# USDA-ARS-GBRU/itsxpress

Measured on AMD Instinct MI355X. Metric: reads/sec trimmed (ITS2, stand-in taxon Tracheophyta for Fungi), higher is better.
Workload: dtype u8+f32

## Files before the change

itsxpress_amd/csrc/engine.hip:

```cpp
#include <algorithm>
#include <chrono>
#include <cmath>
#include <cstdio>
#include <cstring>
#include <functional>
#include <map>
#include <memory>
#include <numeric>
#include <atomic>
#include <condition_variable>
#include <mutex>
#include <thread>
#include "detmath.h"
#include "engine.h"
#include "k_api.h"
#include "cluster_multi.h"
#include "fastq_io.h"
#include "writers.h"

namespace itsx {
void launch_region_offsets(int64_t npairs, const PairRec *pairs, const int32_t *pref, const int64_t *seg_pair_start,
                           const int64_t *seg_region_start, int64_t *pair_region0, hipStream_t st);
void launch_finalize(itsx_domain *dom, int64_t n, const int64_t *domz, double domE, const int32_t *usample, int P, hipStream_t st);
void launch_positions(const itsx_domain *dom, int64_t n, const int8_t *side, unsigned long long *bl, unsigned long long *br,
// ... 190 lines not shown
    NameList r;
    r.blob.assign(blob.begin() + off[lo], blob.begin() + off[hi]);
    r.off.resize(hi - lo + 1);
    for (size_t i = lo; i <= hi; i++) r.off[i - lo] = off[i] - off[lo];
    return r;
  }
};

template <class T> struct DBuf {
  T *p = nullptr; size_t n = 0, cap = 0;
  int pool_device = -1;
  hipError_t alloc(size_t count, bool exact = false)
  {
    n = count;
    if (count <= cap && p) return hipSuccess;
    static const bool trace = sw_get("ITSX_TRACE_ALLOC") != nullptr;
    if (p) {
      const auto f0 = std::chrono::steady_clock::now();
      defer_free(p, cap * sizeof(T));
      if (trace) fprintf(stderr, "[itsx] free %.3f GB: %.1f ms\n", cap * sizeof(T) / 1073741824.0, std::chrono::duration<double, std::milli>(std::chrono::steady_clock::now() - f0).count());
    }
    p = nullptr; cap = 0;
    if (!count) return hipSuccess;
    if (pool_device >= 0) {
      size_t got = 0;
      if (void *q = pool_take(count * sizeof(T), pool_device, &got)) { p = (T *)q; cap = got / sizeof(T); return hipSuccess; }
    }
    const size_t want = exact ? count : count + count / 8 + 64;
    const auto t0 = std::chrono::steady_clock::now();
    hipError_t e = hipMalloc((void **)&p, want * sizeof(T));
    if (trace) fprintf(stderr, "[itsx] hipMalloc %.3f GB: %.1f ms\n", want * sizeof(T) / 1073741824.0, std::chrono::duration<double, std::milli>(std::chrono::steady_clock::now() - t0).count());
    if (e != hipSuccess) {
      (void)hipGetLastError();
      grave_flush();
      e = hipMalloc((void **)&p, count * sizeof(T));
      if (e != hipSuccess) { p = nullptr; return e; }
      cap = count; return e;
    }
    cap = want;
    return hipSuccess;
  }
  void release() { if (p) defer_free(p, cap * sizeof(T)); p = nullptr; n = 0; cap = 0; }
  ~DBuf() { release(); }
};

struct itsx_ctx {
  int device = 0;
  hipStream_t st = nullptr, st2 = nullptr;
  hipStream_t st_hi = nullptr;
  hipStream_t st3 = nullptr; hipEvent_t ev_s3a = nullptr, ev_s3b = nullptr;
  hipEvent_t ev_a = nullptr, ev_b = nullptr;
  hipEvent_t ev_msv0 = nullptr, ev_msv1 = nullptr, ev_c = nullptr;
  int64_t msv_pre_u0 = -1, next_u0 = -1; int32_t next_U = 0;
  mutable std::string err;
  void set_error(const std::string &m) const { err = m; }
  itsx_stats stats{};

  std::vector<HostProfile> profs;
  int P = 0, G = 0;
  DBuf<DevProfile> d_prof;
  DBuf<uint32_t> d_etab;
  DBuf<int32_t> d_pbias, d_ptec, d_ptbm;
  DBuf<float> d_rtab, d_entab;
  DBuf<ChainRec> sh_chain, sh_bchain;
  DBuf<float> d_flogsum; DBuf<LogTab> d_logtab; DBuf<float> d_btab; bool bound_fold = false;
  std::vector<char> generic_q;

  int64_t N = 0;
  itsx_io::Text h_bases;
  const char *bases_view = "";
  const uint8_t *dev_bases = nullptr;
  static constexpr int NSTAGE = 3;
  void *stage_pin[NSTAGE] = {nullptr, nullptr, nullptr}; DBuf<uint8_t> stage_dev[NSTAGE]; hipEvent_t stage_ev[NSTAGE] = {nullptr, nullptr, nullptr}; size_t stage_cap = 0;
  DBuf<int64_t> w_pk_off; DBuf<int8_t> w_pk_lut; DBuf<int32_t> w_pk_excnt, w_pk_exstart, w_pk_tmp; DBuf<long long> w_pk_bad;
  std::vector<int64_t> h_off;
  NameList h_names;
  std::vector<int64_t> h_woff;
  std::vector<int32_t> h_len;
  DBuf<uint32_t> d_words, d_exc;
  DBuf<int64_t> d_woff, d_excoff;
  DBuf<int32_t> d_len;
  ReadsDev rd{};
  int Lmax = 0;
  int32_t S = 1, sel_sample = -1;
  std::vector<int32_t> h_sample, h_usample;
  DBuf<int32_t> d_sample, d_usample;
  const int32_t *dev_sample() const { return S > 1 ? d_sample.p : nullptr; }
  const int32_t *dev_usample() const { return S > 1 ? d_usample.p : nullptr; }
  int32_t usample(int64_t u) const { return S > 1 ? h_usample[(size_t)u] : 0; }
  double slab_gb = 0.0;

  bool have_derep = false;
  std::vector<int32_t> order_cache; bool order_cache_ok = false;
  int derep_strand_both = 1;
  int32_t U = 0;
  int32_t U_active = 0;
  DBuf<int32_t> d_rep_of, d_uniq_of, d_seed_read, d_abund, d_sorted_uniq, d_ulen;
  DBuf<int8_t> d_strand;
  std::vector<int32_t> h_rep_of, h_uniq_of, h_seed_read, h_abund, h_sorted_uniq;
  std::vector<int8_t> h_strand;
  DBuf<uint32_t> d_orient_db; bool have_orient_db = false;
  bool clustered = false;
  std::vector<double> h_pct;
  std::vector<int32_t> h_order;

  bool have_search = false, have_final = false;
  double T = 10.0;
  int64_t npairs_padded = 0;
  DBuf<PairRec> d_pairs;
  DBuf<PairOut> d_pout;
  DBuf<RegionRec> d_regions;
  DBuf<RegionOut> d_rout;
  DBuf<int64_t> d_pair_region0;
  DBuf<int32_t> d_upos;
  DBuf<RegionRec> d_ulist;
  std::vector<std::unique_ptr<DBuf<itsx_domain>>> dom_bufs;
  std::vector<int64_t> dom_n;
  int64_t pair_budget = 0; int32_t trace_u0 = 0; int n_chunks = 0; bool keep_trace = false, trace_sorted = false;
  DBuf<int16_t> d_vtab; DBuf<VitOut> d_vit; bool have_vit = false; double F2 = 1e-6;
  DBuf<int32_t> d_domz32;
  DBuf<int64_t> d_domz64; bool domz_on_device = false;
  bool compact_rows = false; double compact_zmax = 1e9, compact_dome_min = 1e-2, compact_lnp = 0; int compact_ncls = 0;
  DBuf<itsx_domain> w_domscratch; DBuf<int8_t> w_cls; DBuf<unsigned long long> w_bestc; DBuf<int32_t> w_keep, w_keeppos, w_keeptmp;
  int64_t rows_before_compaction = 0;
  int rows_mode = -1;
  bool lazy = false;
  bool domz_exchanged = false;
  int64_t lazy_pending = 0;
  double sF1 = 1e-6, sF3 = 1e-6;
  std::vector<int64_t> domz_ub;
  std::vector<int64_t> domz_loc, domz_ub_loc;
  bool completing = false;
  std::vector<int32_t> h_plist; DBuf<int32_t> d_plist;
  int64_t s_Uc = 0; int s_Lcap = 0;
  DBuf<float> l_fb; DBuf<uint32_t> l_b10; DBuf<uint8_t> l_done; DBuf<int32_t> l_flag, l_pos, l_scan, l_has; DBuf<unsigned long long> l_gtop, l_sure;
  DBuf<PairRec> l_pairs; DBuf<int64_t> l_seg, l_zub; DBuf<int32_t> l_pflag; DBuf<uint8_t> l_uflag; bool partial_coords = false; bool kept_rows = false; std::vector<int32_t> lazy_pending_prof;
  std::vector<uint16_t> thr_memo; std::vector<char> thr_memo_have; double thr_memo_F1 = -1.0; int thr_memo_Ppad = 0;
  DBuf<int32_t> w_coords4; DBuf<int64_t> w_keys128; DBuf<uint64_t> w_hf1, w_hr1;
  std::vector<int32_t> h_sorted_active;
  DBuf<LenTables> d_lt;
  std::vector<int64_t> domz;
  std::vector<itsx_domain> h_dom;
  std::vector<itsx_pairtrace> h_trace;

  DBuf<uint64_t> w_hf, w_hr; DBuf<unsigned long long> w_keys; DBuf<int32_t> w_vals, w_is_seed, w_seed_rank, w_scan_tmp, w_hist, w_cursor, w_tmp2;
  DBuf<uint32_t> w_slot_of; DBuf<unsigned int> w_ncoll;
  DBuf<uint16_t> w_thr, w_res; DBuf<int32_t> w_tjb, w_cnt, w_total, w_rows, w_rcnt, w_rpref, w_scan2, w_b, w_rrows;
  DBuf<int64_t> w_seg_start, w_idx, w_rseg, w_dz, w_counters, w_useg;
  DBuf<int32_t> w_rrep, w_ruq, w_rurank;
  DBuf<WaveDesc> w_waves, w_rw; DBuf<RegionRec> w_raw; DBuf<float> w_slab, w_eslab;
  DBuf<int32_t> w_mrcnt, w_mroff, w_mrlen, w_mrloff, w_mrrows, w_mrulist, w_mrulist2, w_mru; DBuf<int64_t> w_mrrowoff; DBuf<MrRec> w_mr; DBuf<MrOut> w_mrout; DBuf<int64_t> w_n2off; DBuf<float> w_n2sc, w_mrslab;
  DBuf<uint8_t> w_mrscratch; DBuf<WaveDesc> w_mrwaves;
  DBuf<RegionRec> w_pool, w_pool_sorted; DBuf<int32_t> w_pool_k; DBuf<unsigned long long> w_pool_n, w_pool_key; int64_t pool_cap = 0;
  DBuf<int32_t> w_mrsel; DBuf<int64_t> w_mrselrow; DBuf<MrBig> w_mrbig; DBuf<uint8_t> w_mrarena; DBuf<int32_t> w_mrenv; DBuf<WaveDesc> w_mrbigwaves;
  DBuf<int32_t> w_cl, w_cr;
  DBuf<int8_t> w_side; DBuf<unsigned long long> w_bl, w_br; DBuf<int32_t> w_uind, w_us, w_ue, w_ut, w_rs, w_re, w_rt, w_ri, w_uflag;

  struct ShareBatch { int32_t k0, k1; int64_t node0, nnodes; int32_t nsplit; int64_t gnode0, gnnodes; };
  bool share_on = false; int share_B = 32, share_logB = 5, share_maxd = 0;
  DBuf<unsigned long long> sh_tab, sh_mask_s, sh_mask, sh_counters; DBuf<uint8_t> sh_depth_s, sh_depth;
  DBuf<int32_t> sh_src, sh_parent_s, sh_parent, sh_nn_s, sh_nn, sh_node0_s, sh_node0, sh_order, sh_ulen, sh_uorder, sh_inv, sh_flag, sh_pos, sh_bstart, sh_cursor, sh_segk, sh_scan, sh_cuts;
  std::vector<ShareBatch> sh_batches; std::vector<int32_t> sh_segk_h;
  DBuf<uint4> sh_mgslots; size_t sh_mgslots_half = 0;
  DBuf<uint4> sh_mslots; size_t sh_mslots_half = 0, sh_fslots_half = 0; DBuf<uint32_t> sh_pass, sh_need; DBuf<int32_t> sh_real, sh_segflat, sh_segdepth, sh_wc, sh_woff; DBuf<int64_t> sh_bnd;
  DBuf<uint16_t> sh_res_chk; DBuf<float> sh_fb_chk;
  ShareDev sh_dev{};
  std::string switches_at_search;
  struct TopUp { bool valid = false; int64_t NP = 0; std::vector<int64_t> seg_start; std::vector<int32_t> total; int32_t u0 = 0, Uc = 0; } topup;
  DBuf<unsigned long long> l_zneed, l_zsplit, l_tcnt; DBuf<int32_t> l_slot, l_pslot; DBuf<uint32_t> l_cut;
  std::vector<unsigned long long> h_zneed;
  bool prev_lazy = false; int prev_P = 0; int64_t prev_U = 0, prev_Uc = 0;
  std::vector<int32_t> h_merge_index;
  bool two_on = false; int share_maxrd = 0; int32_t Ub = 0; size_t sh_gslots_off = 0;
  DBuf<uint8_t> sh_rdepth_s, sh_rdepth; DBuf<unsigned long long> sh_rmask_s, sh_rmask, sh_keys, sh_keys2;
  DBuf<int32_t> sh_rparent_s, sh_rparent, sh_jlev_s, sh_jown_s, sh_endrow_s, sh_rsteps_s, sh_rnn_s, sh_rnode0_s, sh_endrow, sh_jlev, sh_jsrc, sh_jownb;
  DBuf<int32_t> sh_border_s, sh_invb, sh_bsegk, sh_rnn, sh_rnode0, sh_border, sh_bulen, sh_rsrc, sh_bsteps, sh_vals;
  DBuf<uint8_t> sh_sorttmp;
  std::vector<int32_t> sh_bsegk_h;
  BShareDev sh_bdev{};
  DBuf<uint32_t> sh_needb; DBuf<uint16_t> sh_resb; DBuf<int32_t> sh_cntb, sh_totalb, sh_realb, sh_bsegflat, sh_bsegdepth, sh_bwc, sh_bwoff; DBuf<int64_t> sh_bbnd, sh_bseg_start;
  DBuf<PairRec> sh_bpairs; DBuf<WaveDesc> sh_bwaves;
};

#define CTXCHK(c)                                   \
  if (!(c)) return ITSX_E_ARG;
#define SET_ERR(ctx, code, msg) do { (ctx)->set_error(msg); return (code); } while (0)
#undef HIPCHK
#define HIPCHK(expr)                                                                      \
  do {                                                                                    \
    hipError_t e__ = (expr);                                                              \
    if (e__ != hipSuccess) { ctx->set_error(std::string(#expr) + ": " + hipGetErrorString(e__)); return ITSX_E_DEVICE; } \
  } while (0)

template <class T> static hipError_t upload(DBuf<T> &d, const std::vector<T> &h, hipStream_t st, size_t min_elems = 1)
{
  hipError_t e = d.alloc(std::max(h.size(), min_elems));
  if (e != hipSuccess) return e;
  if (h.empty()) return hipSuccess;
  return hipMemcpyAsync(d.p, h.data(), h.size() * sizeof(T), hipMemcpyHostToDevice, st);
}

struct LazyTimers {
  struct Rec { hipEvent_t a, b; float *acc; };
  std::vector<Rec> recs; hipStream_t st;
  explicit LazyTimers(hipStream_t s) : st(s) {}
  size_t begin(float *acc) { Rec r; (void)hipEventCreate(&r.a); (void)hipEventCreate(&r.b); r.acc = acc; (void)hipEventRecord(r.a, st); recs.push_back(r); return recs.size() - 1; }
  void end(size_t i) { (void)hipEventRecord(recs[i].b, st); }
  void collect()
  {
    for (auto &r : recs) { (void)hipEventSynchronize(r.b); float ms = 0; (void)hipEventElapsedTime(&ms, r.a, r.b); *r.acc += ms; (void)hipEventDestroy(r.a); (void)hipEventDestroy(r.b); }
    recs.clear();
  }
  ~LazyTimers() { collect(); }
};

struct StageTimer {
  hipEvent_t a = nullptr, b = nullptr; hipStream_t st;
  explicit StageTimer(hipStream_t s) : st(s) { (void)hipEventCreate(&a); (void)hipEventCreate(&b); (void)hipEventRecord(a, st); }
  float stop() { (void)hipEventRecord(b, st); (void)hipEventSynchronize(b); float ms = 0; (void)hipEventElapsedTime(&ms, a, b); return ms; }
  ~StageTimer() { if (a) (void)hipEventDestroy(a); if (b) (void)hipEventDestroy(b); }
};

using itsx_io::on_threads;

extern "C" {

int itsx_abi_version(void) { return ITSX_ABI_VERSION; }

const char *itsx_last_error(const itsx_ctx *ctx) { return ctx ? ctx->err.c_str() : g_create_error.c_str(); }

struct LoadPriority {
  itsx_ctx *c; bool on;
  explicit LoadPriority(itsx_ctx *ctx) : c(ctx), on(ctx && ctx->st_hi != nullptr) { if (on) std::swap(c->st, c->st_hi); }
  ~LoadPriority() { if (on) { (void)hipStreamSynchronize(c->st); std::swap(c->st, c->st_hi); } }
  LoadPriority(const LoadPriority &) = delete;
  LoadPriority &operator=(const LoadPriority &) = delete;
};

itsx_ctx *itsx_create(int device_id, int flags)
{
  (void)flags;
  int ndev = 0;
  hipError_t e = hipGetDeviceCount(&ndev);
  if (e != hipSuccess || ndev <= 0) { g_create_error = "no HIP device is visible (the engine has no CPU fallback)"; return nullptr; }
  if (device_id < 0 || device_id >= ndev) { g_create_error = "device ordinal out of range"; return nullptr; }
  e = hipSetDevice(device_id);
  if (e != hipSuccess) { g_create_error = std::string("hipSetDevice: ") + hipGetErrorString(e); return nullptr; }
  hipDeviceProp_t prop;
  if (hipGetDeviceProperties(&prop, device_id) != hipSuccess) { g_create_error = "hipGetDeviceProperties failed"; return nullptr; }
  if (std::string(prop.gcnArchName).compare(0, 6, "gfx950") != 0) {
    g_create_error = std::string("device is ") + prop.gcnArchName + "; this engine ships gfx950 code only";
    return nullptr;
  }
  itsx_ctx *ctx = new itsx_ctx();
  ctx->device = device_id;
  ctx->w_slab.pool_device = device_id;
  { std::lock_guard<std::mutex> g(g_pool_mu); g_live_contexts++; }
  if (hipStreamCreate(&ctx->st) != hipSuccess) { g_create_error = "hipStreamCreate failed"; delete ctx; return nullptr; }
  if (!(sw_get("ITSX_LOAD_PRIORITY") && atoi(sw_get("ITSX_LOAD_PRIORITY")) == 0)) {
    int least = 0, greatest = 0;
    if (hipDeviceGetStreamPriorityRange(&least, &greatest) != hipSuccess || greatest == least ||
        hipStreamCreateWithPriority(&ctx->st_hi, hipStreamDefault, greatest) != hipSuccess) { (void)hipGetLastError(); ctx->st_hi = nullptr; }
  }
  std::vector<float> tbl(16000);
  for (int i = 0; i < 16000; i++) tbl[i] = (float)log(1. + exp((double)-i / 1000.f));
  if (upload(ctx->d_flogsum, tbl, ctx->st) != hipSuccess) { g_create_error = "device allocation failed"; delete ctx; return nullptr; }
  std::vector<LogTab> lt(LOGTAB_N);
  build_logtab(lt.data());
  if (upload(ctx->d_logtab, lt, ctx->st) != hipSuccess) { g_create_error = "device allocation failed"; delete ctx; return nullptr; }
  (void)hipStreamSynchronize(ctx->st);
  return ctx;
}

void itsx_destroy(itsx_ctx *ctx)
{
  if (!ctx) return;
  (void)hipSetDevice(ctx->device);
  (void)hipStreamSynchronize(ctx->st);
  if (ctx->st3) { (void)hipStreamSynchronize(ctx->st3); (void)hipStreamDestroy(ctx->st3); (void)hipEventDestroy(ctx->ev_s3a); (void)hipEventDestroy(ctx->ev_s3b); }
  if (ctx->st2) { (void)hipStreamSynchronize(ctx->st2); (void)hipStreamDestroy(ctx->st2); (void)hipEventDestroy(ctx->ev_a); (void)hipEventDestroy(ctx->ev_b);
                  if (ctx->ev_msv0) { (void)hipEventDestroy(ctx->ev_msv0); (void)hipEventDestroy(ctx->ev_msv1); (void)hipEventDestroy(ctx->ev_c); } }
  (void)hipStreamDestroy(ctx->st);
  if (ctx->st_hi) { (void)hipStreamSynchronize(ctx->st_hi); (void)hipStreamDestroy(ctx->st_hi); }
  for (int k = 0; k < itsx_ctx::NSTAGE; k++) { if (ctx->stage_pin[k]) (void)hipHostFree(ctx->stage_pin[k]); if (ctx->stage_ev[k]) (void)hipEventDestroy(ctx->stage_ev[k]); }
  delete ctx;
  grave_flush();
  bool last = false;
  { std::lock_guard<std::mutex> g(g_pool_mu); last = --g_live_contexts <= 0; }
  if (last) pool_flush();
}

int itsx_release_scratch(itsx_ctx *ctx)
{
  CTXCHK(ctx);
  HIPCHK(hipSetDevice(ctx->device));
  HIPCHK(hipStreamSynchronize(ctx->st));
  if (ctx->st2) HIPCHK(hipStreamSynchronize(ctx->st2));
  if (ctx->st3) HIPCHK(hipStreamSynchronize(ctx->st3));
  if (ctx->w_slab.p) { pool_put(ctx->w_slab.p, ctx->w_slab.cap * sizeof(float), ctx->device); ctx->w_slab.p = nullptr; ctx->w_slab.n = ctx->w_slab.cap = 0; }
  return ITSX_OK;
}

static int install_profiles(itsx_ctx *ctx, std::vector<HostProfile> &pv, int *n_profiles)
{
  for (auto &p : pv) {
    if (p.M > MMAX || p.Q > QMAX) SET_ERR(ctx, ITSX_E_UNSUPPORTED, "model '" + p.name + "' has more than 46 nodes; the device kernels hold at most 46");
// ... 1515 lines not shown
  DBuf<itsx_domain> &d_dom = ctx->compact_rows ? ctx->w_domscratch : *ctx->dom_bufs[di];
  if (NP == 0) return ITSX_OK;
  StageTimer tm_list(st);
  std::vector<WaveDesc> waves; std::vector<char> wgeneric; std::vector<int32_t> rows;
  { const int rc = build_waves(ctx, pl, waves, wgeneric, rows); if (rc != ITSX_OK) return rc; }
  const int NW = (int)waves.size();
  DBuf<WaveDesc> &d_waves = ctx->w_waves;
  S.ms_msv += tm_list.stop();

  if (ctx->slab_gb <= 0.0) {
    ctx->slab_gb = 16.0;
    size_t fr = 0, tot = 0;
    if (hipMemGetInfo(&fr, &tot) == hipSuccess) ctx->slab_gb = std::min(64.0, std::max(1.0, (double)fr / (double)(1ull << 30) / 4.0));
  }
  double slab_gb = ctx->slab_gb;
  if (const char *e = sw_get("ITSX_SLAB_GB")) slab_gb = std::max(0.25, atof(e));
  {
    size_t fr = 0, tot = 0;
    if (hipMemGetInfo(&fr, &tot) == hipSuccess) {
      const double room = ((double)fr / 4.0 + (double)ctx->w_slab.cap * 4.0) / (double)(1ull << 30);
      if (slab_gb > room) { slab_gb = std::max(0.0625, room); S.n_slab_shrinks++; }
    }
  }
  const int64_t row_bytes = 12 * 64 * 4;
  int64_t budget_rows = (int64_t)(slab_gb * (1 << 30)) / row_bytes;
  static const bool adapt = !(sw_get("ITSX_SLAB_ADAPT") && atoi(sw_get("ITSX_SLAB_ADAPT")) == 0);
  if (adapt && !sw_get("ITSX_SLAB_GB")) {
    int64_t total_rows = 0;
    for (int w = 0; w < NW; w++) total_rows += rows[(size_t)w];
    const int64_t floor_rows = ((int64_t)4 << 30) / row_bytes, have_rows = (int64_t)(ctx->w_slab.cap / (12 * 64));
    const int64_t want_rows = std::max(total_rows / 8 + 1, floor_rows);
    budget_rows = std::min(budget_rows, 2 * have_rows >= want_rows ? have_rows : want_rows);
  }
  DBuf<RegionRec> &d_raw = ctx->w_raw;
  HIPCHK(d_raw.alloc((size_t)NP * MAXDOM));
  if (ctx->pool_cap <= 0) ctx->pool_cap = 1 << 16;
  RegionPoolView pv{nullptr, nullptr, 0};
 pool_retry:
  HIPCHK(ctx->w_pool.alloc((size_t)ctx->pool_cap)); HIPCHK(ctx->w_pool_k.alloc((size_t)ctx->pool_cap)); HIPCHK(ctx->w_pool_n.alloc(2));
  HIPCHK(hipMemsetAsync(ctx->w_pool_n.p, 0, 2 * sizeof(unsigned long long), st));
  const itsx_stats stats_before = S;
  {
    StageTimer tm(st);
    struct Batch { int w0, w1; int64_t r; };
    std::vector<Batch> batches;
    DBuf<float> &d_slab = ctx->w_slab;
    for (;;) {
      batches.clear();
      int64_t rmax = 0;
      for (int w0 = 0; w0 < NW;) {
        int w1 = w0; int64_t r = 0;
        while (w1 < NW && wgeneric[w1] == wgeneric[w0] && (w1 == w0 || r + rows[w1] <= budget_rows)) { waves[w1].slab = r; waves[w1].rows = rows[w1]; r += rows[w1]; w1++; }
        batches.push_back(Batch{w0, w1, r});
        rmax = std::max(rmax, r);
        w0 = w1;
      }
      const int64_t slab_rows = batches.size() > 1 ? std::max(rmax, budget_rows) : rmax;
      if ((size_t)slab_rows * 12 * 64 <= d_slab.cap) break;
      if (d_slab.alloc((size_t)slab_rows * 12 * 64, true) == hipSuccess) break;
      (void)hipGetLastError();
      if (budget_rows <= ((int64_t)64 << 20) / row_bytes) SET_ERR(ctx, ITSX_E_NOMEM, "not even 64 MB of device memory are left for the DP slab");
      budget_rows = std::max<int64_t>(budget_rows / 2, ((int64_t)64 << 20) / row_bytes);
      ctx->slab_gb = std::min(ctx->slab_gb, (double)(budget_rows * row_bytes) / (double)(1 << 30));
      S.n_slab_shrinks++;
    }
    HIPCHK(hipMemcpyAsync(d_waves.p, waves.data(), (size_t)NW * sizeof(WaveDesc), hipMemcpyHostToDevice, st));
    FloatArgs a{};
    a.rd = ctx->rd; a.sorted_uniq = d_sorted; a.seed_read = ctx->d_seed_read.p; a.prof = ctx->d_prof.p; a.lt = ctx->d_lt.p;
    a.flogsum = ctx->d_flogsum.p; a.logtab = ctx->d_logtab.p; a.pairs = pl.pairs; a.pout = pl.pout; a.waves = d_waves.p; a.slab = d_slab.p;
    a.regions = d_raw.p; a.F1 = F1; a.F3 = F3;
    a.pool.rec = ctx->w_pool.p; a.pool.k = ctx->w_pool_k.p; a.pool.n = ctx->w_pool_n.p; a.pool.cap = ctx->pool_cap;
    VitArgs va{};
    if (ctx->have_vit) {
      HIPCHK(ctx->d_vit.alloc((size_t)NP));
      va.rd = ctx->rd; va.sorted_uniq = d_sorted; va.seed_read = ctx->d_seed_read.p; va.prof = ctx->d_prof.p; va.lt = ctx->d_lt.p;
      va.pairs = pl.pairs; va.pout = pl.pout; va.waves = d_waves.p; va.vtab = ctx->d_vtab.p; va.vit = ctx->d_vit.p; va.F2 = ctx->F2;
      va.eloop = (int32_t)roundf((float)(500.0 / 0.69314718055994529) * logf(0.5f));
      a.vit = ctx->d_vit.p;
    }
    static const bool overlap = !(sw_get("ITSX_BIAS_OVERLAP") && atoi(sw_get("ITSX_BIAS_OVERLAP")) == 0);
    if (overlap && !ctx->st2) {
      int least = 0, greatest = 0;
      (void)hipDeviceGetStreamPriorityRange(&least, &greatest);
      if (sw_get("ITSX_ST2_PRIO") && atoi(sw_get("ITSX_ST2_PRIO")) == 0) least = 0;
      HIPCHK(hipStreamCreateWithPriority(&ctx->st2, hipStreamNonBlocking, least));
      HIPCHK(hipEventCreateWithFlags(&ctx->ev_a, hipEventDisableTiming)); HIPCHK(hipEventCreateWithFlags(&ctx->ev_b, hipEventDisableTiming));
    }
    LazyTimers lazy(st), lazy2(overlap ? ctx->st2 : st);
    auto bias_batch = [&](const Batch &bt, hipStream_t s, LazyTimers &lz) {
      int w = bt.w0;
      while (w < bt.w1) {
        int e = w + 1;
        while (e < bt.w1 && waves[(size_t)e].first == waves[(size_t)e - 1].first + 64) e++;
        FloatArgs ab = a;
        ab.pairs = pl.pairs + waves[(size_t)w].first; ab.pout = pl.pout + waves[(size_t)w].first;
        const size_t t = lz.begin(&S.ms_bias_kernel); launch_bias(ab, (int64_t)(e - w) * 64, s); lz.end(t);
        w = e;
      }
    };
    if (!batches.empty()) bias_batch(batches[0], st, lazy);
    for (size_t bi = 0; bi < batches.size(); bi++) {
      const Batch &bt = batches[bi];
      const int w0 = bt.w0, w1 = bt.w1;
      a.slab_plane = bt.r * 6 * 64;
      const bool more = bi + 1 < batches.size();
      if (ctx->have_vit) { const size_t t = lazy.begin(&S.ms_vit_kernel); launch_vit(va, w1 - w0, w0, st); lazy.end(t); }
      { const size_t t = lazy.begin(&S.ms_fwd_kernel); launch_filters_fwd(a, w1 - w0, w0, wgeneric[w0], st); lazy.end(t); }
      { const size_t t = lazy.begin(&S.ms_bwd_kernel); launch_bwd_decode(a, w1 - w0, w0, wgeneric[w0], st); lazy.end(t); }
      if (more && overlap) {
        HIPCHK(hipEventRecord(ctx->ev_a, st)); HIPCHK(hipStreamWaitEvent(ctx->st2, ctx->ev_a, 0));
        bias_batch(batches[bi + 1], ctx->st2, lazy2);
        HIPCHK(hipEventRecord(ctx->ev_b, ctx->st2));
      }
      { const size_t t = lazy.begin(&S.ms_decode_kernel); launch_decode(a, w1 - w0, w0, st); lazy.end(t); }
      if (more && overlap) HIPCHK(hipStreamWaitEvent(st, ctx->ev_b, 0));
      else if (more) bias_batch(batches[bi + 1], st, lazy);
      for (int w = w0; w < w1; w++) S.fwd_rows += (int64_t)(rows[w] - 1) * waves[w].count;
      S.n_batches++;
    }
    lazy2.collect();
    lazy.collect();
    S.ms_filters += tm.stop();
  }
  {
    unsigned long long pn = 0;
    HIPCHK(hipMemcpyAsync(&pn, ctx->w_pool_n.p, sizeof(pn), hipMemcpyDeviceToHost, st));
    HIPCHK(hipStreamSynchronize(st));
    if ((int64_t)pn > ctx->pool_cap) {
      while (ctx->pool_cap < (int64_t)pn) ctx->pool_cap *= 2;
      const float keep_ms = S.ms_filters;
      S = stats_before; S.ms_filters = keep_ms; S.n_slab_shrinks++;
      goto pool_retry;
    }
    if (pn > 0) {
      std::vector<RegionRec> hr((size_t)pn); std::vector<int32_t> hk((size_t)pn);
      HIPCHK(hipMemcpyAsync(hr.data(), ctx->w_pool.p, (size_t)pn * sizeof(RegionRec), hipMemcpyDeviceToHost, st));
      HIPCHK(hipMemcpyAsync(hk.data(), ctx->w_pool_k.p, (size_t)pn * 4, hipMemcpyDeviceToHost, st));
      HIPCHK(hipStreamSynchronize(st));
      std::vector<size_t> ord((size_t)pn);
      std::iota(ord.begin(), ord.end(), (size_t)0);
      auto key = [&](size_t i) { return ((unsigned long long)(uint32_t)hr[i].pair << 24) | (unsigned long long)(uint32_t)hk[i]; };
      std::sort(ord.begin(), ord.end(), [&](size_t x, size_t y) { return key(x) < key(y); });
      std::vector<RegionRec> sr((size_t)pn); std::vector<unsigned long long> sk((size_t)pn);
      for (size_t i = 0; i < (size_t)pn; i++) { sr[i] = hr[ord[i]]; sk[i] = key(ord[i]); }
      HIPCHK(upload(ctx->w_pool_sorted, sr, st)); HIPCHK(upload(ctx->w_pool_key, sk, st));
      HIPCHK(hipStreamSynchronize(st));
      pv.rec = ctx->w_pool_sorted.p; pv.key = ctx->w_pool_key.p; pv.n = (int64_t)pn;
    }
  }
  if (next_msv) { const int rc = (*next_msv)(); if (rc != ITSX_OK) return rc; }
  StageTimer tm_dom(st);
  int64_t NMR = 0;
  const bool ensemble = !(sw_get("ITSX_NO_ENSEMBLE") && atoi(sw_get("ITSX_NO_ENSEMBLE")) != 0);
  if (ensemble) {
    DBuf<int32_t> &mrcnt = ctx->w_mrcnt, &mroff = ctx->w_mroff, &stmp = ctx->w_scan2;
    HIPCHK(mrcnt.alloc((size_t)NP + 2)); HIPCHK(mroff.alloc((size_t)NP + 2)); HIPCHK(stmp.alloc((size_t)scan_tmp_elems(NP + 2)));
    launch_mr_count(pl.pout, d_raw.p, pv, NP, mrcnt.p, st);
    launch_exclusive_scan(mrcnt.p, mroff.p, NP + 1, stmp.p, st);
    int32_t tot = 0;
    HIPCHK(hipMemcpyAsync(&tot, mroff.p + NP, 4, hipMemcpyDeviceToHost, st));
    HIPCHK(hipStreamSynchronize(st));
    NMR = tot;
    if (NMR > 0) {
      StageTimer tm_e(st);
      static_assert(sizeof(MrRec) == sizeof(RegionRec), "MrRec is handed to the region memoisation kernels as a RegionRec");
      HIPCHK(ctx->w_mr.alloc((size_t)NMR));
      launch_mr_fill(pl.pout, d_raw.p, pv, NP, mroff.p, ctx->w_mr.p, st);
      DBuf<unsigned long long> &rkeys = ctx->w_keys; DBuf<int32_t> &rvals = ctx->w_vals; DBuf<uint32_t> &rslot = ctx->w_slot_of;
      DBuf<int32_t> &rrep = ctx->w_rrep, &ruq = ctx->w_ruq, &rurank = ctx->w_rurank, &rscan = ctx->w_scan_tmp;
      uint64_t tsize = 1024; while (tsize < (uint64_t)NMR * 2 + 16) tsize <<= 1;
      HIPCHK(rkeys.alloc(tsize)); HIPCHK(rvals.alloc(tsize)); HIPCHK(rslot.alloc((size_t)NMR + 1));
      HIPCHK(rrep.alloc((size_t)NMR + 1)); HIPCHK(ruq.alloc((size_t)NMR + 1)); HIPCHK(rurank.alloc((size_t)NMR + 1)); HIPCHK(rscan.alloc((size_t)scan_tmp_elems(NMR + 1)));
      HIPCHK(hipMemsetAsync(rkeys.p, 0, tsize * sizeof(unsigned long long), st));
      HIPCHK(hipMemsetAsync(rvals.p, 0x7f, tsize * sizeof(int32_t), st));
      HIPCHK(hipMemsetAsync(ruq.p, 0, ((size_t)NMR + 1) * sizeof(int32_t), st));
      const RegionRec *mr_as_regions = (const RegionRec *)ctx->w_mr.p;
      launch_region_keys(ctx->rd, mr_as_regions, NMR, pl.pairs, d_sorted, ctx->d_seed_read.p, rkeys.p, rvals.p, tsize - 1, rslot.p, st);
      launch_region_resolve(ctx->rd, mr_as_regions, NMR, pl.pairs, d_sorted, ctx->d_seed_read.p, rvals.p, rslot.p, rrep.p, ruq.p, st);
      launch_exclusive_scan(ruq.p, rurank.p, NMR + 1, rscan.p, st);
      int32_t NU = 0;
      HIPCHK(hipMemcpyAsync(&NU, rurank.p + NMR, 4, hipMemcpyDeviceToHost, st));
      HIPCHK(hipStreamSynchronize(st));
      DBuf<int32_t> &ulist0 = ctx->w_mrulist, &ulist = ctx->w_mrulist2, &ulen = ctx->w_mrlen, &newpos = ctx->w_mrloff, &mru = ctx->w_mru;
      HIPCHK(ulist0.alloc((size_t)NU + 1)); HIPCHK(ulist.alloc((size_t)NU + 1)); HIPCHK(ulen.alloc((size_t)NU + 2)); HIPCHK(newpos.alloc((size_t)NU + 2)); HIPCHK(mru.alloc((size_t)NMR + 1));
      launch_mr_ulist(NMR, ctx->w_mr.p, rrep.p, ruq.p, rurank.p, ulist0.p, ulen.p, mru.p, st);
      std::vector<int32_t> hlen((size_t)NU), ord((size_t)NU), hpos((size_t)NU);
      HIPCHK(hipMemcpyAsync(hlen.data(), ulen.p, (size_t)NU * 4, hipMemcpyDeviceToHost, st));
      HIPCHK(hipStreamSynchronize(st));
      std::iota(ord.begin(), ord.end(), 0);
      std::stable_sort(ord.begin(), ord.end(), [&](int32_t x, int32_t y) { return hlen[(size_t)x] < hlen[(size_t)y]; });
      std::vector<int64_t> hn2((size_t)NU + 1, 0), hrow((size_t)NU + 1, 0);
      for (int32_t x = 0; x < NU; x++) {
        const int32_t o = ord[(size_t)x];
        hpos[(size_t)o] = x;
        hn2[(size_t)x + 1] = hn2[(size_t)x] + hlen[(size_t)o];
        hrow[(size_t)x + 1] = hrow[(size_t)x] + hlen[(size_t)o] + 1;
      }
      HIPCHK(hipMemcpyAsync(newpos.p, hpos.data(), (size_t)NU * 4, hipMemcpyHostToDevice, st));
      launch_mr_reorder(NU, NMR, newpos.p, ulist0.p, ulist.p, mru.p, st);
      HIPCHK(upload(ctx->w_n2off, hn2, st)); HIPCHK(upload(ctx->w_mrrowoff, hrow, st));
      HIPCHK(ctx->w_mrout.alloc((size_t)NU)); HIPCHK(ctx->w_n2sc.alloc((size_t)hn2[(size_t)NU] + 1));
      static const int lanes_long = sw_get("ITSX_MR_LONG_LANES") ? std::max(1, std::min(MR_LANES, atoi(sw_get("ITSX_MR_LONG_LANES")))) : MR_LANES_LONG;
      static const double frac_long = sw_get("ITSX_MR_LONG_FRAC") ? atof(sw_get("ITSX_MR_LONG_FRAC")) : MR_LONG_FRAC;
      const int64_t n_long = std::min<int64_t>(NU, (int64_t)(frac_long * (double)NU));
      const int64_t waves_target = sw_get("ITSX_MR_WAVES") ? atoll(sw_get("ITSX_MR_WAVES")) : 4096;
      const int lanes_norm = waves_target <= 0 ? MR_LANES : (int)std::max<int64_t>(2, std::min<int64_t>(MR_LANES, (NU + waves_target - 1) / waves_target));
      std::vector<WaveDesc> mw;
      std::vector<int64_t> wfirst;
      for (int64_t x = 0; x < NU;) {
        const int lanes = x >= NU - n_long ? std::min(lanes_long, lanes_norm) : (int)std::min<int64_t>(lanes_norm, NU - n_long - x);
        WaveDesc d{};
        d.prof = -1; d.first = x; d.count = (int32_t)std::min<int64_t>(lanes, (int64_t)NU - x);
        d.rows = hlen[(size_t)ord[(size_t)(d.first + d.count - 1)]] + 1;
        wfirst.push_back(x);
        mw.push_back(d);
        x += d.count;
      }
      const int NMW = (int)mw.size();
      wfirst.push_back(NU);
      HIPCHK(upload(ctx->w_mrwaves, mw, st));
      const int64_t mrow_bytes = (int64_t)MRV * 16;
      const int64_t mbudget = std::max<int64_t>(1, (int64_t)(std::min(slab_gb, 16.0) * (1 << 30)) / mrow_bytes);
      const int64_t wave_cap = std::max<int64_t>(1, ((int64_t)6 << 30) / ((int64_t)MR_SCRATCH * MR_LANES));
      int w0 = 0;
      int64_t mr_wave_cap = wave_cap;
      while (w0 < NMW) {
        int w1 = w0;
        const int64_t row0 = hrow[(size_t)wfirst[(size_t)w0]];
        auto rows_to = [&](int w) { return hrow[(size_t)wfirst[(size_t)std::min(w, NMW)]] - row0; };
        while (w1 < NMW && w1 - w0 < std::min(wave_cap, mr_wave_cap) && (w1 == w0 || rows_to(w1 + 1) <= mbudget)) w1++;
        const int64_t r = rows_to(w1);
        if (((size_t)r * MRV * 4 > ctx->w_mrslab.cap && ctx->w_mrslab.alloc((size_t)r * MRV * 4) != hipSuccess) ||
            ctx->w_mrscratch.alloc((size_t)(wfirst[(size_t)w1] - wfirst[(size_t)w0]) * MR_SCRATCH) != hipSuccess) {
          (void)hipGetLastError();
          if (w1 - w0 <= 1) SET_ERR(ctx, ITSX_E_NOMEM, "no device memory left for the matrices of one wave of multidomain regions");
          mr_wave_cap = std::max<int64_t>(1, (int64_t)(w1 - w0) / 2);
          S.n_slab_shrinks++;
          continue;
        }
        MrArgs ma{};
        ma.rd = ctx->rd; ma.sorted_uniq = d_sorted; ma.seed_read = ctx->d_seed_read.p; ma.prof = ctx->d_prof.p; ma.pairs = pl.pairs;
        ma.mr = ctx->w_mr.p; ma.ulist = ulist.p; ma.u0 = wfirst[(size_t)w0]; ma.waves = ctx->w_mrwaves.p; ma.slab = (float4 *)ctx->w_mrslab.p;
        ma.rowoff = ctx->w_mrrowoff.p; ma.rowoff0 = row0;
        ma.n2off = ctx->w_n2off.p; ma.n2sc = ctx->w_n2sc.p; ma.out = ctx->w_mrout.p; ma.scratch = ctx->w_mrscratch.p;
        static const bool mrdbg = sw_get("ITSX_MR_DEBUG") != nullptr;
        if (mrdbg) { HIPCHK(ctx->w_counters.alloc(8)); HIPCHK(hipMemsetAsync(ctx->w_counters.p, 0, 64, st)); ma.dbg = (unsigned long long *)ctx->w_counters.p; }
        const int64_t one_max = sw_get("ITSX_MR_ONE_MAX") ? atoll(sw_get("ITSX_MR_ONE_MAX")) : 2048;
        const int64_t nreg = wfirst[(size_t)w1] - wfirst[(size_t)w0];
        const bool one = nreg <= one_max;
        if (one) ma.lds_bytes = (int32_t)std::min<int64_t>(40 << 10, (int64_t)mw[(size_t)w1 - 1].rows * MRV * 16);
        launch_mr_ensemble(ma, w1 - w0, w0, st, one ? wfirst[(size_t)w0] : 0, one ? nreg : 0);
        if (mrdbg) {
          unsigned long long d[5];
          HIPCHK(hipMemcpyAsync(d, ctx->w_counters.p, 40, hipMemcpyDeviceToHost, st)); HIPCHK(hipStreamSynchronize(st));
          fprintf(stderr, "[itsx] ensemble batch: %d waves, %lld matrix rows; per wave (100 MHz ticks): walk %.0f, close %.0f (samples %.0f), cluster %.0f\n", w1 - w0, (long long)r,
                  (double)d[0] / std::max<double>(1.0, (double)d[3]), (double)d[1] / std::max<double>(1.0, (double)d[3]), (double)d[4] / std::max<double>(1.0, (double)d[3]),
                  (double)d[2] / std::max<double>(1.0, (double)d[3]));
        }
        w0 = w1;
      }
      {
        HIPCHK(ctx->w_mrsel.alloc((size_t)NU + 1)); HIPCHK(ctx->w_pool_n.alloc(2));
        HIPCHK(hipMemsetAsync(ctx->w_pool_n.p + 1, 0, sizeof(unsigned long long), st));
        launch_mr_overflowed(ctx->w_mrout.p, NU, ctx->w_mrsel.p, ctx->w_pool_n.p + 1, st);
        unsigned long long nov = 0;
        HIPCHK(hipMemcpyAsync(&nov, ctx->w_pool_n.p + 1, sizeof(nov), hipMemcpyDeviceToHost, st));
        HIPCHK(hipStreamSynchronize(st));
        if (nov > 0) {
          std::vector<int32_t> sel((size_t)nov);
          HIPCHK(hipMemcpyAsync(sel.data(), ctx->w_mrsel.p, (size_t)nov * 4, hipMemcpyDeviceToHost, st));
          HIPCHK(hipStreamSynchronize(st));
          std::sort(sel.begin(), sel.end());
          S.n_mr_overflow += (int64_t)nov;
          int64_t envtot = 0;
          std::vector<int64_t> envoff(sel.size());
          for (size_t x = 0; x < sel.size(); x++) { envoff[x] = envtot; envtot += 8 * ((int64_t)hlen[(size_t)ord[(size_t)sel[x]]] + 1); }
          HIPCHK(ctx->w_mrenv.alloc((size_t)envtot + 8));
          size_t x0 = 0;
          while (x0 < sel.size()) {
            std::vector<MrBig> big; std::vector<int64_t> srow; std::vector<WaveDesc> bw;
            int64_t arena = 0, rows = 0; size_t x1 = x0;
            while (x1 < sel.size()) {
              const int Lr = hlen[(size_t)ord[(size_t)sel[x1]]];
              MrBig g{}; g.capD = Lr + 1; g.capT = 200 * g.capD;
              uint32_t hs = 1024; while (hs < 2u * (uint32_t)g.capT) hs <<= 1;
              g.hmask = hs - 1;
              auto al = [](int64_t v) { return (v + 15) & ~(int64_t)15; };
              const int64_t capSig = 4 * (int64_t)g.capD;
              const int64_t bytes = al(8ll * g.capT) + 6 * al(4ll * g.capT) + al(4ll * hs) + al(4ll * g.capD) + al(16ll * g.capD) + 3 * al(4 * capSig) +
                                    al(g.capT) + al(2ll * g.capD) + al(capSig) + al(2 * MR_EPC) + 64;
              g.envoff = envoff[x1];
              if (x1 > x0 && arena + bytes > ((int64_t)8 << 30)) break;
              g.off = arena; arena += bytes;
              big.push_back(g); srow.push_back(rows); rows += Lr + 1;
              x1++;
            }
            for (size_t x = x0; x < x1; x += MR_LANES_LONG) {
              WaveDesc d{}; d.prof = -1; d.first = (int64_t)(x - x0); d.count = (int32_t)std::min<size_t>(MR_LANES_LONG, x1 - x);
              d.rows = hlen[(size_t)ord[(size_t)sel[x + d.count - 1]]] + 1;
              bw.push_back(d);
            }
            std::vector<int32_t> selb(sel.begin() + x0, sel.begin() + x1);
            HIPCHK(upload(ctx->w_mrsel, selb, st)); HIPCHK(upload(ctx->w_mrselrow, srow, st)); HIPCHK(upload(ctx->w_mrbig, big, st)); HIPCHK(upload(ctx->w_mrbigwaves, bw, st));
            if ((size_t)rows * MRV * 4 > ctx->w_mrslab.cap) HIPCHK(ctx->w_mrslab.alloc((size_t)rows * MRV * 4));
            HIPCHK(ctx->w_mrarena.alloc((size_t)arena));
            MrArgs mb{};
            mb.rd = ctx->rd; mb.sorted_uniq = d_sorted; mb.seed_read = ctx->d_seed_read.p; mb.prof = ctx->d_prof.p; mb.pairs = pl.pairs;
            mb.mr = ctx->w_mr.p; mb.ulist = ulist.p; mb.u0 = 0; mb.waves = ctx->w_mrbigwaves.p; mb.slab = (float4 *)ctx->w_mrslab.p;
            mb.rowoff = ctx->w_mrrowoff.p; mb.rowoff0 = 0; mb.n2off = ctx->w_n2off.p; mb.n2sc = ctx->w_n2sc.p; mb.out = ctx->w_mrout.p;
            mb.scratch = nullptr; mb.sel = ctx->w_mrsel.p; mb.sel_rowoff = ctx->w_mrselrow.p; mb.big = ctx->w_mrbig.p; mb.arena = ctx->w_mrarena.p; mb.envpool = ctx->w_mrenv.p;
            launch_mr_ensemble_big(mb, (int)bw.size(), st);
            x0 = x1;
          }
        }
      }
      S.ms_ensemble += tm_e.stop();
      HIPCHK(hipGetLastError());
      S.n_mr_clustered += NMR; S.n_mr_distinct += NU;
    }
  }
  DBuf<int32_t> &d_rcnt = ctx->w_rcnt, &d_rpref = ctx->w_rpref, &d_scan_tmp = ctx->w_scan2;
  HIPCHK(d_rcnt.alloc((size_t)NP + 1)); HIPCHK(d_rpref.alloc((size_t)NP + 1)); HIPCHK(d_scan_tmp.alloc((size_t)scan_tmp_elems(NP + 1)));
  HIPCHK(hipMemsetAsync(d_rcnt.p, 0, ((size_t)NP + 1) * 4, st));
  RegionListArgs rl{};
  rl.pout = pl.pout; rl.raw = d_raw.p; rl.pv = pv; rl.npairs = NP;
  if (NMR > 0) { rl.mr_off = ctx->w_mroff.p; rl.mr_u = ctx->w_mru.p; rl.mrout = ctx->w_mrout.p; rl.envpool = ctx->w_mrenv.p; }
  {
    DBuf<int64_t> &d_c = ctx->w_counters;
    HIPCHK(d_c.alloc(16));
    HIPCHK(hipMemsetAsync(d_c.p, 0, 16 * sizeof(int64_t), st));
    launch_region_list_count(rl, d_rcnt.p, (unsigned long long *)d_c.p, st);
    int64_t hc[10] = {0};
    HIPCHK(hipMemcpyAsync(hc, d_c.p, sizeof(hc), hipMemcpyDeviceToHost, st));
    HIPCHK(hipStreamSynchronize(st));
    S.n_mr_failed += hc[0]; S.n_mr_envelopes += hc[1];
    for (int k = 0; k < 8; k++) S.n_mr_fail_kind[k] += hc[2 + k];
  }
  launch_exclusive_scan(d_rcnt.p, d_rpref.p, NP + 1, d_scan_tmp.p, st);
  std::vector<int32_t> bound((size_t)P + 1);
  {
    DBuf<int64_t> &d_idx = ctx->w_idx; DBuf<int32_t> &d_b = ctx->w_b;
    HIPCHK(upload(d_idx, pl.seg_start, st)); HIPCHK(d_b.alloc((size_t)P + 1));
    hipLaunchKernelGGL(k_gather_i32, dim3((P + 1 + 255) / 256), dim3(256), 0, st, d_rpref.p, d_idx.p, P + 1, d_b.p);
    HIPCHK(hipMemcpyAsync(bound.data(), d_b.p, ((size_t)P + 1) * 4, hipMemcpyDeviceToHost, st));
    HIPCHK(hipStreamSynchronize(st));
  }
  std::vector<int64_t> rseg((size_t)P + 1, 0);
  std::vector<int32_t> rtotal((size_t)P);
  for (int p = 0; p < P; p++) { rtotal[p] = bound[p + 1] - bound[p]; rseg[p + 1] = rseg[p] + ((int64_t)rtotal[p] + 63) / 64 * 64; S.n_domains += rtotal[p]; }
  const int64_t NR = rseg[P];
  ctx->dom_n[di] = NR;
  HIPCHK(ctx->d_pair_region0.alloc((size_t)NP));
  HIPCHK(ctx->d_regions.alloc((size_t)std::max<int64_t>(NR, 1)));
  HIPCHK(d_dom.alloc((size_t)std::max<int64_t>(NR, 1)));
  HIPCHK(hipMemsetAsync(d_dom.p, 0xFF, (size_t)std::max<int64_t>(NR, 1) * sizeof(itsx_domain), st));
  if (NR > 0) {
    DBuf<int64_t> &d_rseg = ctx->w_rseg;
    HIPCHK(upload(d_rseg, rseg, st));
    launch_region_offsets(NP, pl.pairs, d_rpref.p, pl.d_seg_start, d_rseg.p, ctx->d_pair_region0.p, st);
    HIPCHK(hipMemsetAsync(ctx->d_regions.p, 0xFF, (size_t)NR * sizeof(RegionRec), st));
    launch_region_list_fill(rl, ctx->d_pair_region0.p, ctx->d_regions.p, st);
    DBuf<unsigned long long> &rkeys = ctx->w_keys; DBuf<int32_t> &rvals = ctx->w_vals; DBuf<uint32_t> &rslot = ctx->w_slot_of;
    DBuf<int32_t> &rrep = ctx->w_rrep, &ruq = ctx->w_ruq, &rurank = ctx->w_rurank, &rscan = ctx->w_scan_tmp;
    uint64_t tsize = 1024; while (tsize < (uint64_t)NR * 2 + 16) tsize <<= 1;
    HIPCHK(rkeys.alloc(tsize)); HIPCHK(rvals.alloc(tsize)); HIPCHK(rslot.alloc((size_t)NR + 1));
    HIPCHK(rrep.alloc((size_t)NR + 1)); HIPCHK(ruq.alloc((size_t)NR + 1)); HIPCHK(rurank.alloc((size_t)NR + 1));
    HIPCHK(rscan.alloc((size_t)scan_tmp_elems(NR + 1))); HIPCHK(ctx->d_upos.alloc((size_t)NR + 1));
    HIPCHK(hipMemsetAsync(rkeys.p, 0, tsize * sizeof(unsigned long long), st));
    HIPCHK(hipMemsetAsync(rvals.p, 0x7f, tsize * sizeof(int32_t), st));
    HIPCHK(hipMemsetAsync(ruq.p, 0, ((size_t)NR + 1) * sizeof(int32_t), st));
    launch_region_keys(ctx->rd, ctx->d_regions.p, NR, pl.pairs, d_sorted, ctx->d_seed_read.p, rkeys.p, rvals.p, tsize - 1, rslot.p, st);
    launch_region_resolve(ctx->rd, ctx->d_regions.p, NR, pl.pairs, d_sorted, ctx->d_seed_read.p, rvals.p, rslot.p, rrep.p, ruq.p, st);
    launch_exclusive_scan(ruq.p, rurank.p, NR + 1, rscan.p, st);
    std::vector<int32_t> ub((size_t)P + 1);
    {
      DBuf<int64_t> &d_idx = ctx->w_idx; DBuf<int32_t> &d_b = ctx->w_b;
      HIPCHK(upload(d_idx, rseg, st)); HIPCHK(d_b.alloc((size_t)P + 1));
      hipLaunchKernelGGL(k_gather_i32, dim3((P + 1 + 255) / 256), dim3(256), 0, st, rurank.p, d_idx.p, P + 1, d_b.p);
      HIPCHK(hipMemcpyAsync(ub.data(), d_b.p, ((size_t)P + 1) * 4, hipMemcpyDeviceToHost, st));
      HIPCHK(hipStreamSynchronize(st));
    }
    std::vector<int64_t> useg((size_t)P + 1, 0);
    std::vector<int32_t> utotal((size_t)P);
    for (int p = 0; p < P; p++) { utotal[p] = ub[p + 1] - ub[p]; useg[p + 1] = useg[p] + ((int64_t)utotal[p] + 63) / 64 * 64; S.n_env_unique += utotal[p]; }
    const int64_t NU = useg[P];
    DBuf<int64_t> &d_useg = ctx->w_useg;
    HIPCHK(upload(d_useg, useg, st));
    HIPCHK(ctx->d_ulist.alloc((size_t)std::max<int64_t>(NU, 1))); HIPCHK(ctx->d_rout.alloc((size_t)std::max<int64_t>(NU, 1)));
    HIPCHK(hipMemsetAsync(ctx->d_rout.p, 0, (size_t)std::max<int64_t>(NU, 1) * sizeof(RegionOut), st));
    launch_region_upos(NR, ctx->d_regions.p, pl.pairs, ruq.p, rurank.p, d_rseg.p, d_useg.p, ctx->d_upos.p, ctx->d_ulist.p, st);
    launch_region_upos_follow(NR, rrep.p, ruq.p, ctx->d_upos.p, st);
    std::vector<WaveDesc> rw; std::vector<char> rgen;
    for (int pass = 0; pass < 2; pass++)
      for (int p = 0; p < P; p++) {
        if ((int)ctx->generic_q[p] != pass) continue;
        for (int64_t k = 0; k < utotal[p]; k += 64) {
          WaveDesc w{}; w.prof = p; w.first = useg[p] + k; w.count = (int32_t)std::min<int64_t>(64, utotal[p] - k);
          rw.push_back(w); rgen.push_back((char)pass);
        }
      }
    const int NRW = (int)rw.size();
    DBuf<WaveDesc> &d_rw = ctx->w_rw; DBuf<int32_t> &d_rrows = ctx->w_rrows;
    HIPCHK(upload(d_rw, rw, st)); HIPCHK(d_rrows.alloc((size_t)NRW));
    hipLaunchKernelGGL(k_wave_rows_regions, dim3((NRW + 255) / 256), dim3(256), 0, st, d_rw.p, NRW, ctx->d_ulist.p, d_rrows.p);
    std::vector<int32_t> rrows((size_t)NRW);
    HIPCHK(hipMemcpyAsync(rrows.data(), d_rrows.p, (size_t)NRW * 4, hipMemcpyDeviceToHost, st));
    HIPCHK(hipStreamSynchronize(st));
    const int64_t erow_bytes = 104 * 64 * 4;
    int64_t ebudget = (int64_t)(slab_gb * (1 << 30)) / erow_bytes;
    LazyTimers elazy(st);
    DBuf<float> &d_eslab = ctx->w_eslab; int64_t ealloc = (int64_t)(d_eslab.cap / (104 * 64));
    if (adapt && !sw_get("ITSX_SLAB_GB")) {
      int64_t total_rows = 0;
      for (int w = 0; w < NRW; w++) total_rows += rrows[(size_t)w];
      ebudget = std::min(ebudget, std::max(std::max(total_rows / 4 + 1, ((int64_t)2 << 30) / erow_bytes), ealloc));
    }
    int w0 = 0;
    while (w0 < NRW) {
      int w1 = w0; int64_t r = 0;
      while (w1 < NRW && rgen[w1] == rgen[w0] && (w1 == w0 || r + rrows[w1] <= ebudget)) { rw[w1].slab = r; rw[w1].rows = rrows[w1]; r += rrows[w1]; w1++; }
      if (r > ealloc) {
        if (d_eslab.alloc((size_t)r * 104 * 64) != hipSuccess) {
          (void)hipGetLastError();
          ealloc = 0;
          if (w1 - w0 <= 1) SET_ERR(ctx, ITSX_E_NOMEM, "no device memory left for the envelope slab of a single wave");
          ebudget = std::max<int64_t>(r / 2, rrows[(size_t)w0]);
          S.n_slab_shrinks++;
          continue;
        }
        ealloc = r;
      }
      HIPCHK(hipMemcpyAsync(d_rw.p + w0, rw.data() + w0, (size_t)(w1 - w0) * sizeof(WaveDesc), hipMemcpyHostToDevice, st));
      EnvArgs a{};
      a.rd = ctx->rd; a.sorted_uniq = d_sorted; a.seed_read = ctx->d_seed_read.p; a.prof = ctx->d_prof.p; a.lt = ctx->d_lt.p;
      a.pairs = pl.pairs; a.regions = ctx->d_ulist.p; a.rout = ctx->d_rout.p; a.waves = d_rw.p; a.slab = d_eslab.p;
      { const size_t t = elazy.begin(&S.ms_env_kernel); launch_envelopes(a, w1 - w0, w0, rgen[w0], st); elazy.end(t); }
      for (int w = w0; w < w1; w++) S.env_rows += (int64_t)(rrows[w] - 1) * rw[w].count;
      w0 = w1;
    }
    ScoreArgs sa{};
    sa.rd = ctx->rd; sa.sorted_uniq = d_sorted; sa.seed_read = ctx->d_seed_read.p; sa.prof = ctx->d_prof.p; sa.lt = ctx->d_lt.p;
    sa.flogsum = ctx->d_flogsum.p; sa.pairs = pl.pairs; sa.pout = pl.pout; sa.regions = ctx->d_regions.p; sa.rout = ctx->d_rout.p;
    sa.pair_region0 = ctx->d_pair_region0.p; sa.upos = ctx->d_upos.p; sa.dom = d_dom.p; sa.npairs = NP; sa.T = T;
    if (NMR > 0) { sa.mr = ctx->w_mr.p; sa.mr_u = ctx->w_mru.p; sa.mrout = ctx->w_mrout.p; sa.n2off = ctx->w_n2off.p; sa.n2sc = ctx->w_n2sc.p; sa.mr_off = ctx->w_mroff.p; }
    sa.domz = ctx->d_domz32.p; sa.usample = ctx->dev_usample(); sa.P = ctx->P;
    launch_score(sa, st);
    if (ctx->compact_rows) {
      launch_compact_best(d_dom.p, NR, ctx->w_cls.p, ctx->compact_ncls, ctx->compact_lnp, ctx->w_bestc.p, st);
      HIPCHK(ctx->w_keep.alloc((size_t)NR + 1)); HIPCHK(ctx->w_keeppos.alloc((size_t)NR + 1)); HIPCHK(ctx->w_keeptmp.alloc((size_t)scan_tmp_elems(NR + 1)));
      launch_compact_mark(d_dom.p, NR, ctx->w_cls.p, ctx->compact_ncls, ctx->compact_lnp, ctx->w_bestc.p, ctx->w_keep.p, st);
      launch_exclusive_scan(ctx->w_keep.p, ctx->w_keeppos.p, NR + 1, ctx->w_keeptmp.p, st);
      int32_t kept = 0;
      HIPCHK(hipMemcpyAsync(&kept, ctx->w_keeppos.p + NR, sizeof(kept), hipMemcpyDeviceToHost, st));
      HIPCHK(hipStreamSynchronize(st));
      DBuf<itsx_domain> &small = *ctx->dom_bufs[di];
      HIPCHK(small.alloc((size_t)std::max<int32_t>(kept, 1), true));
      launch_compact_scatter(d_dom.p, NR, ctx->w_keep.p, ctx->w_keeppos.p, small.p, st);
      ctx->rows_before_compaction += NR;
      ctx->dom_n[di] = kept;
    }
  }
  S.ms_domains += tm_dom.stop();
  {
    DBuf<int64_t> &d_c = ctx->w_counters;
    HIPCHK(d_c.alloc(8));
    HIPCHK(hipMemsetAsync(d_c.p, 0, 8 * sizeof(int64_t), st));
    hipLaunchKernelGGL(k_pair_counters, dim3((unsigned)std::min<int64_t>(4096, (NP + 255) / 256)), dim3(256), 0, st, pl.pout, NP, (unsigned long long *)d_c.p);
    int64_t hc[8];
    HIPCHK(hipMemcpyAsync(hc, d_c.p, sizeof(hc), hipMemcpyDeviceToHost, st));
    HIPCHK(hipStreamSynchronize(st));
    S.n_past_bias += hc[0]; S.n_past_fwd += hc[1]; S.n_regions += hc[2]; S.n_domain_overflow += hc[3]; S.n_multidomain += hc[4];
  }
  HIPCHK(hipGetLastError());
  return ITSX_OK;
}


namespace itsx {
__global__ void k_dbg_group_count(const PairRec *__restrict__ pairs, int64_t NP, const int32_t *__restrict__ flag, const int8_t *__restrict__ cls, int ncls, unsigned long long *__restrict__ cnt)
{
  const int64_t i = (int64_t)blockIdx.x * blockDim.x + threadIdx.x;
  if (i >= NP || !flag[i]) return;
  const PairRec pr = pairs[i];
  if (pr.prof < 0) return;
  atomicAdd(&cnt[(size_t)pr.useq * ncls + cls[pr.prof]], 1ull);
}
__global__ void k_dbg_group_hist(const unsigned long long *__restrict__ cnt, int64_t ng, unsigned long long *__restrict__ hist)
{
  const int64_t i = (int64_t)blockIdx.x * blockDim.x + threadIdx.x;
  if (i >= ng) return;
  const unsigned long long c = cnt[i];
  const int b = c <= 4 ? (int)c : c <= 8 ? 5 : c <= 16 ? 6 : 7;
  atomicAdd(&hist[b], 1ull);
  if (c > 1) atomicAdd(&hist[8], c - 1);
  if (c > 2) atomicAdd(&hist[9], c - 2);
}
}

static int lazy_rounds(itsx_ctx *ctx, const PairList &pl, const int32_t *d_sorted, int32_t u0, int32_t Uc, double T, double F1, double F3, const std::function<int()> *next_msv)
{
  hipStream_t st = ctx->st;
  const int P = ctx->P, ncls = ctx->compact_ncls;
  itsx_stats &S = ctx->stats;
  const int64_t NP = pl.NP;
  HIPCHK(ctx->l_fb.alloc((size_t)NP + 1)); HIPCHK(ctx->l_b10.alloc((size_t)NP + 1)); HIPCHK(ctx->l_done.alloc((size_t)NP + 1));
  HIPCHK(ctx->l_flag.alloc((size_t)NP + 2)); HIPCHK(ctx->l_pos.alloc((size_t)NP + 2)); HIPCHK(ctx->l_scan.alloc((size_t)scan_tmp_elems(NP + 2)));
  HIPCHK(ctx->l_gtop.alloc((size_t)Uc * ncls + 1));
  HIPCHK(hipMemsetAsync(ctx->l_done.p, 0, (size_t)NP + 1, st));
  HIPCHK(hipMemsetAsync(ctx->l_gtop.p, 0, ((size_t)Uc * ncls + 1) * sizeof(unsigned long long), st));
  if (ctx->share_on) {
    const int maxd = ctx->share_maxd, DS = maxd + 1;
    const bool two = ctx->two_on;
    std::vector<int32_t> segflat, segdepth, segbatch;
    for (size_t bi = 0; bi < ctx->sh_batches.size(); bi++) {
      const auto &b = ctx->sh_batches[bi];
      if (b.k0 < u0 || b.k0 >= u0 + Uc) continue;
      for (int d = 0; d < DS; d++) { segflat.push_back(ctx->sh_segk_h[bi * SHARE_SEGS + d] - u0); segdepth.push_back(d); segbatch.push_back((int32_t)bi); }
    }
    const int nseg = (int)segdepth.size();
    segflat.push_back(Uc);
    if ((int64_t)nseg * P + 1 >= (1ll << 31)) SET_ERR(ctx, ITSX_E_UNSUPPORTED, "prefix sharing: too many (batch, depth, profile) segments in one chunk");
    HIPCHK(upload(ctx->sh_segflat, segflat, st)); HIPCHK(upload(ctx->sh_segdepth, segdepth, st, 1)); HIPCHK(upload(ctx->w_rcnt, pl.total, st));
    HIPCHK(ctx->sh_bnd.alloc((size_t)(nseg + 1) * P)); HIPCHK(ctx->sh_wc.alloc((size_t)nseg * P + 2)); HIPCHK(ctx->sh_woff.alloc((size_t)nseg * P + 2));
    HIPCHK(ctx->sh_scan.alloc((size_t)scan_tmp_elems((int64_t)nseg * P + 2)));
    launch_share_bounds(pl.pairs, pl.d_seg_start, ctx->w_rcnt.p, ctx->sh_segflat.p, nseg, P, ctx->sh_bnd.p, st);
    launch_share_wcount(ctx->sh_bnd.p, nseg, P, ctx->sh_wc.p, st);
    launch_exclusive_scan(ctx->sh_wc.p, ctx->sh_woff.p, (int64_t)nseg * P + 1, ctx->sh_scan.p, st);
    std::vector<int32_t> woff((size_t)nseg * P + 1);
    HIPCHK(hipMemcpyAsync(woff.data(), ctx->sh_woff.p, woff.size() * 4, hipMemcpyDeviceToHost, st));
    HIPCHK(hipStreamSynchronize(st));
    const int NW = woff.back();
    HIPCHK(ctx->w_waves.alloc((size_t)std::max(NW, 1))); HIPCHK(ctx->w_counters.alloc(512));
    HIPCHK(hipMemsetAsync(ctx->w_counters.p, 0, 512 * sizeof(int64_t), st));
    launch_share_waves(NW, nseg, P, ctx->sh_woff.p, ctx->sh_bnd.p, ctx->sh_segdepth.p, ctx->share_B, pl.pairs, two ? ctx->sh_endrow.p + u0 : nullptr, 0, ctx->w_waves.p,
                       (unsigned long long *)ctx->w_counters.p, st);
    std::vector<int64_t> lr((size_t)384, 0);
    FloatArgs a{};
    a.rd = ctx->rd; a.sorted_uniq = d_sorted; a.seed_read = ctx->d_seed_read.p; a.prof = ctx->d_prof.p; a.lt = ctx->d_lt.p;
    a.pairs = pl.pairs; a.waves = ctx->w_waves.p; a.F1 = F1; a.F3 = F3;
    const int maxrd = ctx->share_maxrd, DSB = maxrd + 1;
    int32_t cb0 = 0, Ubc = 0; int NWB = 0;
    std::vector<int32_t> bwoff;
    FloatArgs ab = a;
    if (two) {
      int32_t cb1 = 0; bool any = false;
      std::vector<int32_t> bsegflat, bsegdepth;
      for (size_t bi = 0; bi < ctx->sh_batches.size(); bi++) {
        const auto &b = ctx->sh_batches[bi];
        if (b.k0 < u0 || b.k0 >= u0 + Uc) continue;
        const int32_t lo = ctx->sh_bsegk_h[bi * SHARE_SEGS], hi = ctx->sh_bsegk_h[bi * SHARE_SEGS + SHARE_SEGS - 1];
        if (!any) { cb0 = lo; any = true; }
        cb1 = hi;
      }
      Ubc = any ? cb1 - cb0 : 0;
      for (size_t bi = 0; bi < ctx->sh_batches.size(); bi++) {
        const auto &b = ctx->sh_batches[bi];
        if (b.k0 < u0 || b.k0 >= u0 + Uc) continue;
        for (int d = 0; d < DSB; d++) { bsegflat.push_back(ctx->sh_bsegk_h[bi * SHARE_SEGS + d] - cb0); bsegdepth.push_back(d); }
      }
      const int nbseg = (int)bsegdepth.size();
      bsegflat.push_back(Ubc);
      bwoff.assign((size_t)nbseg * P + 1, 0);
      if (Ubc > 0) {
        const int W = (P + 31) / 32;
        HIPCHK(ctx->sh_needb.alloc((size_t)Ubc * W + 1));
        HIPCHK(hipMemsetAsync(ctx->sh_needb.p, 0, ((size_t)Ubc * W + 1) * 4, st));
        launch_join_need(ctx->sh_jlev.p + u0, ctx->sh_jownb.p + u0, Uc, W, cb0, ctx->sh_pass.p, ctx->sh_needb.p, st);
        for (int r = maxrd; r >= 1; r--) launch_need_up_b(r, ctx->sh_rdepth.p + cb0, ctx->sh_rparent.p + cb0, cb0, Ubc, W, ctx->sh_needb.p, st);
        HIPCHK(ctx->sh_resb.alloc((size_t)P * Ubc + 1));
        launch_need_res(ctx->sh_needb.p, Ubc, P, W, ctx->sh_resb.p, st);
        const int nchb = (Ubc + CHUNK - 1) / CHUNK;
        HIPCHK(ctx->sh_cntb.alloc((size_t)P * nchb)); HIPCHK(ctx->sh_totalb.alloc((size_t)P)); HIPCHK(ctx->sh_realb.alloc((size_t)P));
        HIPCHK(hipMemsetAsync(ctx->sh_realb.p, 0, (size_t)P * 4, st));
        launch_pair_count(ctx->sh_resb.p, P, Ubc, nchb, ctx->sh_cntb.p, ctx->sh_realb.p, st);
        launch_chunk_scan(ctx->sh_cntb.p, P, nchb, ctx->sh_totalb.p, st);
        std::vector<int32_t> totalb((size_t)P);
        HIPCHK(hipMemcpyAsync(totalb.data(), ctx->sh_totalb.p, (size_t)P * 4, hipMemcpyDeviceToHost, st));
        HIPCHK(hipStreamSynchronize(st));
        std::vector<int64_t> bseg((size_t)P + 1, 0);
        for (int p = 0; p < P; p++) bseg[(size_t)p + 1] = bseg[(size_t)p] + ((int64_t)totalb[(size_t)p] + 63) / 64 * 64;
        const int64_t NPB = bseg[(size_t)P];
        if (NPB >= (1ll << 31) || (int64_t)nbseg * P + 1 >= (1ll << 31)) SET_ERR(ctx, ITSX_E_UNSUPPORTED, "two-sided sharing: too many Backward chains in one chunk");
        if (NPB > 0) {
          HIPCHK(upload(ctx->sh_bseg_start, bseg, st));
          HIPCHK(ctx->sh_bpairs.alloc((size_t)NPB));
          HIPCHK(hipMemsetAsync(ctx->sh_bpairs.p, 0xFF, (size_t)NPB * sizeof(PairRec), st));
          launch_pair_fill(ctx->sh_resb.p, P, Ubc, nchb, ctx->sh_cntb.p, ctx->sh_bseg_start.p, ctx->sh_bulen.p + cb0, ctx->sh_bpairs.p, st);
          HIPCHK(upload(ctx->sh_bsegflat, bsegflat, st)); HIPCHK(upload(ctx->sh_bsegdepth, bsegdepth, st, 1));
          HIPCHK(ctx->sh_bbnd.alloc((size_t)(nbseg + 1) * P)); HIPCHK(ctx->sh_bwc.alloc((size_t)nbseg * P + 2)); HIPCHK(ctx->sh_bwoff.alloc((size_t)nbseg * P + 2));
          HIPCHK(ctx->sh_scan.alloc((size_t)scan_tmp_elems((int64_t)nbseg * P + 2)));
          launch_share_bounds(ctx->sh_bpairs.p, ctx->sh_bseg_start.p, ctx->sh_totalb.p, ctx->sh_bsegflat.p, nbseg, P, ctx->sh_bbnd.p, st);
          launch_share_wcount(ctx->sh_bbnd.p, nbseg, P, ctx->sh_bwc.p, st);
          launch_exclusive_scan(ctx->sh_bwc.p, ctx->sh_bwoff.p, (int64_t)nbseg * P + 1, ctx->sh_scan.p, st);
          HIPCHK(hipMemcpyAsync(bwoff.data(), ctx->sh_bwoff.p, bwoff.size() * 4, hipMemcpyDeviceToHost, st));
          HIPCHK(hipStreamSynchronize(st));
          NWB = bwoff.back();
          HIPCHK(ctx->sh_bwaves.alloc((size_t)std::max(NWB, 1)));
          launch_share_waves(NWB, nbseg, P, ctx->sh_bwoff.p, ctx->sh_bbnd.p, ctx->sh_bsegdepth.p, ctx->share_B, ctx->sh_bpairs.p, ctx->sh_bsteps.p + cb0, 1, ctx->sh_bwaves.p,
                             (unsigned long long *)ctx->w_counters.p + 128, st);
// ... 1583 lines not shown
```

itsxpress_amd/csrc/k_api.h:

```cpp
#pragma once
#include "engine.h"

#include "detmath.h"
namespace itsx {

struct ReadsDev {
  const uint32_t *words;
  const int64_t  *woff;
  const int32_t  *len;
  const int64_t  *excoff;
  const uint32_t *exc;
  int64_t         n;
};

void launch_hash_reads(const ReadsDev &rd, uint64_t seed, int strand_both, uint64_t *hf, uint64_t *hr, hipStream_t st, const int32_t *sample = nullptr);
void launch_table_insert(int64_t n, const int32_t *len, int minlen, const uint64_t *hf, const uint64_t *hr,
                         unsigned long long *keys, int32_t *vals, uint64_t mask, uint32_t *slot_of, hipStream_t st);
void launch_table_resolve(const ReadsDev &rd, const uint64_t *hf, const int32_t *vals, const uint32_t *slot_of,
                          int32_t *rep_of, int8_t *strand, int32_t *is_seed, unsigned int *n_collisions, hipStream_t st,
                          const int32_t *sample = nullptr);
void launch_uniques(int64_t n, const int32_t *rep_of, const int32_t *seed_rank, int32_t *uniq_of, int32_t *seed_read,
                    int32_t *abundance, hipStream_t st);
void launch_len_hist(int32_t U, const int32_t *seed_read, const int32_t *len, int32_t *hist, int32_t lcap, hipStream_t st, int32_t nb = 0 );
void launch_len_scatter(int32_t U, const int32_t *seed_read, const int32_t *len, int32_t *cursor, int32_t lcap,
                        int32_t *sorted_uniq, hipStream_t st, int32_t nb = 0);

void launch_region_keys(const ReadsDev &rd, const RegionRec *regions, int64_t nr, const PairRec *pairs, const int32_t *sorted_uniq,
                        const int32_t *seed_read, unsigned long long *keys, int32_t *vals, uint64_t mask, uint32_t *slot_of, hipStream_t st);
void launch_region_resolve(const ReadsDev &rd, const RegionRec *regions, int64_t nr, const PairRec *pairs, const int32_t *sorted_uniq,
                           const int32_t *seed_read, const int32_t *vals, const uint32_t *slot_of, int32_t *rep_region, int32_t *is_uniq, hipStream_t st);
void launch_region_upos(int64_t nr, const RegionRec *regions, const PairRec *pairs, const int32_t *is_uniq, const int32_t *urank,
                        const int64_t *rseg, const int64_t *useg, int32_t *upos, RegionRec *ulist, hipStream_t st);
void launch_region_upos_follow(int64_t nr, const int32_t *rep_region, const int32_t *is_uniq, int32_t *upos, hipStream_t st);

struct ClusterArgs {
  ReadsDev rd;
  const int32_t *order;
  int32_t nq;
  int32_t strand_both;
  int32_t *cent_len, *cent_pos, *cent_read;
  int32_t *cent_q;
  int32_t G;
  int32_t seg;
  const int32_t *sg_q0, *sg_cb, *sg_base, *sg_C, *sg_pos0;
  int32_t *qpos, *qseg;
  int32_t *newcol;
  int64_t pool0;
  uint16_t *klist; int32_t kcap; int32_t *nk;
  uint16_t *cw_pool; int64_t *cw_off; int32_t *cw_n;
  int32_t *wsum, *wscan;
  int32_t *qi_cnt, *qi_cur, *qi_off; uint16_t *qi_ent;
  int32_t *qi_hid; int32_t *qi_nheavy; uint32_t *qi_bm; int32_t hcap; int32_t heavy_min;
  uint32_t *tq, *minm;
  unsigned long long *tkey;
  unsigned long long *cand; int32_t *ncand; int32_t ccap; int32_t *ovf;
  int32_t *ntop;
  uint16_t *cntx; int32_t xpitch;
  int32_t *state, *rejects, *acc_col;
  unsigned long long *prev, *bound;
  double *acc_id;
  int32_t *sel, *selm, *sel_short; unsigned long long *selkey; double *selpid;
  int32_t *wn, *wcol; unsigned long long *wkey; double *wpid;
  int32_t *res_col; int8_t *res_strand; double *res_id;
  int32_t *is_new, *new_rank;
  int32_t *newq, *rm;
  int32_t *xlist, *xn, *hard; unsigned long long *xkey; double *xpid;
  int32_t *work, *xwork, *work_n;
  int32_t *spairs;
  int32_t *awork;
  const uint32_t *dmask;
  const uint64_t *rhash;
  unsigned long long *ctab_key; int32_t *ctab_val; int32_t *canon;
  int32_t *replay;
  int32_t *skipm;
  int32_t *wout;
  int32_t *dbg;
  unsigned long long *scratch; int32_t scratch_pitch;
  double thr;
  unsigned long long *n_align;
  int32_t *need; int32_t need_pitch;
  unsigned long long *n_skipped;
  unsigned long long *pre_stats;
  int32_t pre_k;
  int32_t use_score;
};
constexpr int CL_QS_MAX = 8192;
constexpr int CL_HEAVY = 128;
void launch_cl_segs(const ClusterArgs &a, hipStream_t st);
void launch_cl_kmers(const ClusterArgs &a, hipStream_t st);
void launch_cl_qindex(const ClusterArgs &a, int32_t *scan_tmp, hipStream_t st);
void launch_cl_stream(const ClusterArgs &a, int c0, int c1, int mode, hipStream_t st);
void launch_cl_topk(const ClusterArgs &a, int final, hipStream_t st);
void launch_cl_init(const ClusterArgs &a, hipStream_t st);
void launch_cl_walk(const ClusterArgs &a, int rows_per_lane, hipStream_t st);
void launch_cl_outcome(const ClusterArgs &a, hipStream_t st);
void launch_cl_wsum(const ClusterArgs &a, hipStream_t st);
void launch_cl_columns(const ClusterArgs &a, int clear, hipStream_t st);
void launch_cl_validate(const ClusterArgs &a, int rows_per_lane, hipStream_t st);
void launch_cl_finalize(int32_t nk, const int32_t *order, const int32_t *res_col, const int8_t *res_strand, const double *res_id,
                        const int32_t *cent_read, int32_t *rep_of, int8_t *strand, double *pct, int32_t *is_seed, hipStream_t st);

void launch_orient(const ReadsDev &rd, const uint32_t *dbbits , const uint32_t *dmask , int8_t *strand, int32_t *cfwd, int32_t *crev, hipStream_t st);
void launch_dust(const ReadsDev &rd, uint32_t *dmask, hipStream_t st);

struct MergeArgs {
  const uint8_t *fseq, *fqual, *rseq, *rqual;
  const int64_t *foff, *roff;
  int64_t n;
  int32_t max_total;
  int32_t maxdiffs, allow_stagger; double maxee;
  const double *q2p, *match, *mism;
  const uint8_t *qsame, *qdiff;
  uint8_t *out_seq, *out_qual;
  int32_t *out_len, *reason, *shift; double *score;
};
void launch_merge(const MergeArgs &a, hipStream_t st);

int64_t scan_tmp_elems(int64_t n);
void    launch_exclusive_scan(const int32_t *in, int32_t *out, int64_t n, int32_t *tmp, hipStream_t st);
void    launch_pack(const uint8_t *raw, int64_t raw_base, const int64_t *off, const int64_t *woff, int64_t r0, int64_t r1, const int8_t *lut,
                    uint32_t *words, int32_t *excnt, long long *first_bad, hipStream_t st);
void    launch_pack_exc(const uint8_t *raw, int64_t raw_base, const int64_t *off, int64_t r0, int64_t r1, const int8_t *lut, const int32_t *excnt,
                        const int32_t *exstart, long long *ebase, int64_t ecap, int64_t *excoff, uint32_t *exc, hipStream_t st);
void    launch_calib(int pattern, float *slab, int64_t nwaves, int64_t R, float *out, hipStream_t st);
void    launch_issue(int op, int waves_per_simd, int iters, int blocks, unsigned long long *ticks, float *sink, hipStream_t st);
void    launch_detmath(const double *x, int64_t n, double *ol, double *oe, hipStream_t st);
void    launch_logf_fast(const float *x, int64_t n, const LogTab *tab, float *out, hipStream_t st);

struct TrieArgs {
  ReadsDev rd;
  const int32_t *sorted_uniq, *seed_read;
  int32_t U, Uc, B;
  int32_t rev;
  unsigned long long *tab; uint64_t tmask;
  uint8_t *depth;
  int32_t *parent;
  unsigned long long *mask;
  int32_t *nn;
  unsigned long long *counters;
};
void launch_trie_keycount(const TrieArgs &a, hipStream_t st);
void launch_trie_insert(const TrieArgs &a, hipStream_t st);
void launch_trie_resolve(const TrieArgs &a, hipStream_t st);
void launch_trie_link(const TrieArgs &a, hipStream_t st);
void launch_trie_count(const TrieArgs &a, hipStream_t st);
void launch_share_cuts(const int32_t *ulen, const int32_t *node0_s, const int32_t *rnode0_s , int32_t U, int32_t Uc, int32_t cap,
                       int32_t *cuts , unsigned long long *n, hipStream_t st);
struct PairRec;
void launch_diff_u16(const uint16_t *x, const uint16_t *y, int64_t n, unsigned long long *c, hipStream_t st);
void launch_diff_scores(const float *x, const float *y, const PairRec *pairs, int64_t n, const int32_t *jlev , unsigned long long *c , hipStream_t st);
void launch_popc64(const unsigned long long *m, int32_t *out, int64_t n, int64_t nvalid, hipStream_t st);
constexpr int SHARE_SEGS = 66;
struct ShareDev {
  uint8_t *depth; int32_t *parent ; unsigned long long *mask; int32_t *nn, *node0; int32_t *order , *ulen;
  int32_t *src;
  int32_t *endrow, *jlev, *jsrc;
};
void launch_share_src(const ShareDev &o, int32_t U, int32_t Uc, hipStream_t st);
struct JoinArgs {
  TrieArgs t;
  const uint8_t *fdepth; const unsigned long long *fmask;
  unsigned long long *rmask;
  int32_t *jlev, *jown;
  int32_t *endrow;
  int32_t *rsteps;
  unsigned long long *counters;
};
void launch_join_resolve(const JoinArgs &a, hipStream_t st);
void launch_join_up(const JoinArgs &a, int r, hipStream_t st);
void launch_join_ends(const JoinArgs &a, hipStream_t st);
void launch_order_keys(const uint8_t *depth, const int32_t *minor, const int32_t *runs , int32_t U, const int32_t *bstart, int nb, unsigned long long *keys, int32_t *vals, hipStream_t st);
size_t order_sort_bytes(int64_t n);
int  order_sort(void *tmp, size_t bytes, const unsigned long long *kin, unsigned long long *kout, const int32_t *vin, int32_t *vout, int64_t n, hipStream_t st);
void launch_order_segk(const unsigned long long *sorted_keys, int32_t n, int nb, int32_t *segk , int32_t *inv , const int32_t *vals, int32_t U, unsigned long long *nvalid, hipStream_t st);
void launch_share_permute(const TrieArgs &a, const int32_t *ulen_s, const int32_t *uorder, const int32_t *inv, const int32_t *endrow_s, const int32_t *jlev_s,
                          const ShareDev &o, hipStream_t st);
struct BShareDev {
  uint8_t *depth; int32_t *parent ; unsigned long long *mask; int32_t *nn, *node0; int32_t *order , *ulen;
  int32_t *src;
  int32_t *steps;
};
void launch_bshare_permute(const TrieArgs &a, int32_t Ub, const int32_t *ulen_s, const int32_t *border_s, const int32_t *invb, const unsigned long long *rmask_s,
                           const int32_t *rsteps_s, const BShareDev &o, hipStream_t st);
void launch_bshare_src(const BShareDev &o, int32_t Ub, hipStream_t st);
void launch_join_src(int32_t U, int32_t B, const int32_t *uorder, const int32_t *jown_s, const int32_t *invb, const BShareDev &ob, const ShareDev &o, int32_t *jownb, hipStream_t st);
void launch_join_need(const int32_t *jlev, const int32_t *jownb, int32_t U, int32_t W, int32_t cb0, const uint32_t *pass, uint32_t *need_b, hipStream_t st);
// ... 46 lines not shown
  const uint16_t *thr;
  const int32_t *tjb;
  int32_t Lcap;
  uint16_t *res;
  const int32_t *plist;
  int32_t nlist;
  int32_t k0, k1;
  int32_t pfirst, plast;
  int32_t wtl;
  int32_t share;
  ShareLaunch sl;
};
void launch_msv(const MsvArgs &a, hipStream_t st, int lds_pad = 0);

constexpr int CHUNK = 2048;
void launch_pair_count(const uint16_t *res, int32_t P, int32_t U, int32_t nchunks, int32_t *cnt , int32_t *real , hipStream_t st);
void launch_chunk_scan(int32_t *cnt, int32_t P, int32_t nchunks, int32_t *total , hipStream_t st);
void launch_pair_fill(const uint16_t *res, int32_t P, int32_t U, int32_t nchunks, const int32_t *cnt,
                      const int64_t *seg_start , const int32_t *ulen ,
                      PairRec *pairs, hipStream_t st);
void launch_fill_ulen(int32_t U, const int32_t *sorted_uniq, const int32_t *seed_read, const int32_t *len, int32_t *ulen, hipStream_t st);

struct WaveDesc {
  int32_t prof;
  int32_t count;
  int64_t first;
  int64_t slab;
  int32_t rows;
  int32_t pad;
};
struct VitOut { float vitsc; int32_t ran, pass; };
struct RegionPool { RegionRec *rec; int32_t *k; unsigned long long *n; int64_t cap; };
__device__ __forceinline__ void pool_put(const RegionPool &p, const RegionRec &r, int k)
{
  const unsigned long long i = atomicAdd(p.n, 1ULL);
  if ((int64_t)i < p.cap) { p.rec[i] = r; p.k[i] = k; }
}
struct RegionPoolView { const RegionRec *rec; const unsigned long long *key; int64_t n; };
__device__ __forceinline__ RegionRec raw_region(const RegionRec *raw, const RegionPoolView &pv, int64_t pi, int k)
{
  if (k < MAXDOM) return raw[pi * MAXDOM + k];
  const unsigned long long want = ((unsigned long long)pi << 24) | (unsigned long long)k;
  int64_t lo = 0, hi = pv.n;
  while (lo < hi) { const int64_t mid = (lo + hi) >> 1; if (pv.key[mid] < want) lo = mid + 1; else hi = mid; }
  return pv.rec[lo];
}
struct FloatArgs {
  ReadsDev rd;
  const int32_t *sorted_uniq, *seed_read;
  const DevProfile *prof;
  const LenTables *lt;
  const float *flogsum;
  const LogTab *logtab;
  const PairRec *pairs;
  PairOut *pout;
  const WaveDesc *waves;
  float *slab;
  int64_t slab_plane;
  RegionRec *regions;
  RegionPool pool;
  const VitOut *vit;
  double F1, F3;
};
struct VitArgs {
  ReadsDev rd;
  const int32_t *sorted_uniq, *seed_read;
  const DevProfile *prof;
  const LenTables *lt;
  const PairRec *pairs;
  const PairOut *pout;
  const WaveDesc *waves;
  const int16_t *vtab;
  VitOut *vit;
  int32_t eloop;
  double F2;
};
void launch_vit(const VitArgs &a, int nwaves, int wave0, hipStream_t st);
void launch_bias(const FloatArgs &a, int64_t npairs, hipStream_t st, int lds_pad = 0);
void launch_filters_fwd(const FloatArgs &a, int nwaves, int wave0, int generic_q, hipStream_t st);
void launch_fwd_bound(const FloatArgs &a, float *fb, int nwaves, int wave0, int generic_q, hipStream_t st);
void launch_fwd_bound_seq(const FloatArgs &a, const float *btab, bool fold, float *fb, int nwaves, int wave0, hipStream_t st);
void launch_fwd_bound_share(const FloatArgs &a, const float *btab, bool fold, float *fb, int nwaves, int wave0, const ShareLaunch &sl, hipStream_t st);
void launch_bwd_bound_share(const FloatArgs &a, const float *btab, const float *rtab, int nwaves, int wave0, const ShareLaunch &sl, hipStream_t st);
void launch_bwd_decode(const FloatArgs &a, int nwaves, int wave0, int generic_q, hipStream_t st);
void launch_decode(const FloatArgs &a, int nwaves, int wave0, hipStream_t st);

struct EnvArgs {
  ReadsDev rd;
  const int32_t *sorted_uniq, *seed_read;
  const DevProfile *prof;
  const LenTables *lt;
  const PairRec *pairs;
  const RegionRec *regions;
  RegionOut *rout;
  const WaveDesc *waves;
  float *slab;
};
void launch_envelopes(const EnvArgs &a, int nwaves, int wave0, int generic_q, hipStream_t st);

constexpr int MRV = 52;
constexpr int MRENV = 4;
#ifndef ITSX_MR_LANES
#define ITSX_MR_LANES 64
#endif
constexpr int MR_LANES = ITSX_MR_LANES;
constexpr int MR_LANES_LONG = 4;
constexpr double MR_LONG_FRAC = 0.02;
constexpr int MR_MAXD = 8;
constexpr int MR_TCAP = 512;
constexpr int MR_SCAP = 200 * MR_MAXD;
constexpr int MR_NSIG = 32;
static_assert(MR_NSIG * 50 >= 200 * MR_MAXD, "MR_NSIG must hold every cluster that can reach 25 % of 200 paths");
constexpr int MR_HASH = 1024;
constexpr int MR_EPC = 256;
constexpr int MR_SCRATCH = 19456;
struct MrRec { int32_t pair, ireg, jreg, slot; };
struct MrOut { int32_t status, nenv; int32_t ei[MRENV], ej[MRENV]; int64_t big; };
struct MrBig { int64_t off, envoff; int32_t capD, capT; uint32_t hmask; int32_t pad; };
struct MrArgs {
  ReadsDev rd;
  const int32_t *sorted_uniq, *seed_read;
  const DevProfile *prof;
  const PairRec *pairs;
  const MrRec *mr;
  const int32_t *ulist;
  int64_t u0;
  const WaveDesc *waves;
  int32_t lds_bytes = 0;
  float4 *slab;
  const int64_t *rowoff;
  int64_t rowoff0;
  const int64_t *n2off;
  float *n2sc;
  MrOut *out;
  uint8_t *scratch;
  const int32_t *sel; const int64_t *sel_rowoff; const MrBig *big; uint8_t *arena;
  int32_t *envpool;
  unsigned long long *dbg;
};
void launch_mr_count(const PairOut *pout, const RegionRec *raw, RegionPoolView pv, int64_t npairs, int32_t *cnt, hipStream_t st);
void launch_mr_fill(const PairOut *pout, const RegionRec *raw, RegionPoolView pv, int64_t npairs, const int32_t *off, MrRec *mr, hipStream_t st);
void launch_mr_ulist(int64_t nmr, const MrRec *mr, const int32_t *rep, const int32_t *is_uniq, const int32_t *urank, int32_t *ulist, int32_t *ulen,
                     int32_t *mr_u, hipStream_t st);
void launch_mr_reorder(int64_t nu, int64_t nmr, const int32_t *newpos, const int32_t *ulist_in, int32_t *ulist_out, int32_t *mr_u, hipStream_t st);
void launch_mr_ensemble(const MrArgs &a, int nwaves, int wave0, hipStream_t st, int64_t one_first = 0, int64_t one_count = 0);
void launch_mr_ensemble_big(const MrArgs &a, int nwaves, hipStream_t st);
void launch_mr_overflowed(const MrOut *out, int64_t nu, int32_t *list, unsigned long long *n, hipStream_t st);
struct RegionListArgs {
  PairOut *pout; const RegionRec *raw; RegionPoolView pv; int64_t npairs;
  const int32_t *mr_off; const int32_t *mr_u; const MrOut *mrout; const int32_t *envpool;
};
void launch_region_list_count(const RegionListArgs &a, int32_t *cnt, unsigned long long *counters, hipStream_t st);
void launch_region_list_fill(const RegionListArgs &a, const int64_t *pair_region0, RegionRec *out, hipStream_t st);

struct ScoreArgs {
  ReadsDev rd;
  const int32_t *sorted_uniq, *seed_read;
  const DevProfile *prof;
  const LenTables *lt;
  const float *flogsum;
  const PairRec *pairs;
  const PairOut *pout;
  const RegionRec *regions;
  const RegionOut *rout;
  const int64_t *pair_region0;
  const int32_t *upos;
  itsx_domain *dom;
  int64_t npairs;
  double T;
  const MrRec *mr; const int32_t *mr_u; const MrOut *mrout; const int64_t *n2off; const float *n2sc; const int32_t *mr_off;
  int32_t *domz;
  const int32_t *usample;
  int32_t P;
};
void launch_score(const ScoreArgs &a, hipStream_t st);
void launch_region_count_fill(const PairOut *pout, const RegionRec *raw, int64_t npairs, const int32_t *pref,
                              const int64_t *seg_pair_start, const int64_t *seg_region_start, const int32_t *seg_of_pair_base,
                              RegionRec *out, hipStream_t st);

__host__ __device__ __forceinline__ unsigned long long rank_key(const itsx_domain &d)
{
  long long tenths = (long long)__builtin_rint((double)d.bitscore * 10.0) + (1ll << 23);
  if (tenths < 0) tenths = 0;
  if (tenths > (1ll << 24) - 1) tenths = (1ll << 24) - 1;
  const unsigned long long di = (unsigned long long)(d.dom_idx < 0 ? 0 : (d.dom_idx > 0xFFFFF ? 0xFFFFF : d.dom_idx));
  return ((unsigned long long)tenths << 40) | ((unsigned long long)(0xFFFFF - (d.prof & 0xFFFFF)) << 20) | (0xFFFFFull - di);
}

constexpr int LAZY_TENTHS_BIAS = 1 << 23;
struct LazyArgs {
  const PairRec *pairs; int64_t NP;
  const float *fb;
  const LenTables *lt;
  const int8_t *cls; int32_t ncls;
  const int32_t *sorted_uniq;
  uint32_t *b10;
  unsigned long long *gtop;
  const unsigned long long *bestc;
  uint8_t *done;
  int32_t *flag;
};
void launch_lazy_bound(const LazyArgs &a, hipStream_t st);
void launch_lazy_mark(const LazyArgs &a, int round, hipStream_t st);
void launch_lazy_scatter(const PairRec *pairs, int64_t NP, const int32_t *flag, const int32_t *pos, const int64_t *seg_old, const int64_t *seg_new,
                         PairRec *out, hipStream_t st);
void launch_finalize_lazy(itsx_domain *dom, int64_t n, const int64_t *zlb, const int64_t *zub, double domE, const int32_t *usample, int P, hipStream_t st);
void launch_lazy_sure(const itsx_domain *dom, int64_t n, const int8_t *cls, int ncls, unsigned long long *sure, int32_t *has, hipStream_t st);
void launch_lazy_pending(const itsx_domain *dom, int64_t n, const int8_t *cls, int ncls, const unsigned long long *sure, const int32_t *has,
                         unsigned long long *count, int32_t *prof_flag, uint8_t *uniq_flag, unsigned long long *zneed , const unsigned long long *zsplit , double domE, hipStream_t st);
void launch_topup_count(const uint8_t *done, const int64_t *seg_start, const int32_t *total, const int32_t *prof_of_slot, int nslots, unsigned long long *cnt, hipStream_t st);
void launch_topup_keys(const PairRec *pairs, int64_t NP, const uint8_t *done, const uint32_t *b10, const int32_t *slot_of_prof, int32_t *flag, const int32_t *pos ,
                       unsigned long long *keys, int32_t *vals, hipStream_t st);
void launch_topup_mark(const PairRec *pairs, int64_t NP, uint8_t *done, const uint32_t *b10, const int32_t *slot_of_prof, const uint32_t *cutoff, int32_t *flag, hipStream_t st);

}
```

itsxpress_amd/csrc/k_derep.hip:

```cpp
#include "engine.h"
#include "k_api.h"

namespace itsx {

static constexpr uint64_t XP1 = 11400714785074694791ULL, XP2 = 14029467366897019727ULL,
                          XP3 = 1609587929392839161ULL, XP4 = 9650029242287828579ULL,
                          XP5 = 2870177450012600261ULL;
__device__ __forceinline__ uint64_t rotl64(uint64_t x, int r) { return (x << r) | (x >> (64 - r)); }
__device__ __forceinline__ uint64_t xround(uint64_t acc, uint64_t in) { acc += in * XP2; acc = rotl64(acc, 31); return acc * XP1; }
__device__ __forceinline__ uint64_t xmerge(uint64_t acc, uint64_t v) { acc ^= xround(0, v); return acc * XP1 + XP4; }

__device__ __forceinline__ uint32_t comp_code(uint32_t c)
{
  const uint64_t lut = 0xFBCDEA9785640123ULL;
  return (uint32_t)(lut >> (4 * c)) & 15u;
}

__device__ __forceinline__ uint32_t rev_fields(uint32_t w)
{
  w = __brev(w);
  return ((w >> 1) & 0x55555555u) | ((w & 0x55555555u) << 1);
}

__device__ __forceinline__ uint32_t rc_word(const uint32_t *__restrict__ w, int L, int nw, int j)
// ... 141 lines not shown
                                                       int32_t *__restrict__ is_seed, unsigned int *__restrict__ n_collisions,
                                                       const int32_t *__restrict__ sample)
{
  for (int64_t r = (int64_t)blockIdx.x * blockDim.x + threadIdx.x; r < rd.n; r += (int64_t)gridDim.x * blockDim.x) {
    const uint32_t slot = slot_of[r];
    if (slot == 0xFFFFFFFFu) { rep_of[r] = -1; strand[r] = 0; is_seed[r] = 0; continue; }
    const int32_t s = vals[slot];
    int8_t st = 0;
    if (s == (int32_t)r) st = 1;
    else if (sample && sample[r] != sample[s]) st = 0;
    else if (hf[r] == hf[s] && same_forward(rd, r, s)) st = 1;
    else if (rc_equals_forward(rd, r, s)) st = -1;
    else if (same_forward(rd, r, s)) st = 1;
    if (st == 0) { atomicAdd(n_collisions, 1u); rep_of[r] = (int32_t)r; strand[r] = 1; is_seed[r] = 1; continue; }
    rep_of[r] = s; strand[r] = st; is_seed[r] = (s == (int32_t)r);
  }
}

__global__ void __launch_bounds__(256) k_uniques(int64_t n, const int32_t *__restrict__ rep_of, const int32_t *__restrict__ seed_rank,
                                                 int32_t *__restrict__ uniq_of, int32_t *__restrict__ seed_read,
                                                 int32_t *__restrict__ abundance)
{
  for (int64_t r = (int64_t)blockIdx.x * blockDim.x + threadIdx.x; r < n; r += (int64_t)gridDim.x * blockDim.x) {
    const int32_t s = rep_of[r];
    if (s < 0) { uniq_of[r] = -1; continue; }
    const int32_t u = seed_rank[s];
    uniq_of[r] = u;
    if (s == (int32_t)r) seed_read[u] = (int32_t)r;
    atomicAdd(&abundance[u], 1);
  }
}

__global__ void __launch_bounds__(256) k_len_hist(int32_t U, const int32_t *__restrict__ seed_read, const int32_t *__restrict__ len,
                                                  int32_t *__restrict__ hist, int32_t lcap)
{
  const int32_t stride = gridDim.x * blockDim.x;
  for (int32_t u0 = blockIdx.x * blockDim.x; u0 < U; u0 += stride) {
    const int32_t u = u0 + threadIdx.x;
    const bool ok = u < U;
    int L = ok ? len[seed_read[u]] : -1; if (L >= lcap) L = lcap - 1;
    unsigned long long todo = __ballot(ok);
    while (todo) {
      const int leader = __ffsll((long long)todo) - 1;
      const int L0 = __shfl(L, leader, 64);
      const unsigned long long same = __ballot(ok && L == L0) & todo;
      if ((int)(threadIdx.x & 63) == leader) atomicAdd(&hist[L0], __popcll(same));
      todo &= ~same;
    }
  }
}
constexpr int LEN_TILE = 4096;
template <bool SCATTER>
__global__ void __launch_bounds__(256) k_len_bins(int32_t U, const int32_t *__restrict__ seed_read, const int32_t *__restrict__ len,
                                                  int32_t *__restrict__ hist_or_cursor, int32_t nb, int32_t *__restrict__ sorted_uniq)
{
  extern __shared__ int32_t lds_bins[];
  int32_t *cnt = lds_bins, *base = lds_bins + nb;
  for (int b = threadIdx.x; b < nb; b += 256) cnt[b] = 0;
  __syncthreads();
  const int32_t u0 = blockIdx.x * LEN_TILE, u1 = min(U, u0 + LEN_TILE);
  int32_t myL[LEN_TILE / 256];
#pragma unroll
  for (int k = 0; k < LEN_TILE / 256; k++) {
    const int32_t u = u0 + k * 256 + (int32_t)threadIdx.x;
    int L = -1;
    if (u < u1) { L = len[seed_read[u]]; if (L >= nb) L = nb - 1; atomicAdd(&cnt[L], 1); }
    myL[k] = L;
  }
  __syncthreads();
  for (int b = threadIdx.x; b < nb; b += 256) {
    const int32_t c = cnt[b];
    if (c) {
      const int32_t g = atomicAdd(&hist_or_cursor[b], c);
      if (SCATTER) { base[b] = g; cnt[b] = 0; }
    }
  }
  if (!SCATTER) return;
  __syncthreads();
#pragma unroll
  for (int k = 0; k < LEN_TILE / 256; k++) {
    const int L = myL[k];
    if (L >= 0) sorted_uniq[base[L] + atomicAdd(&cnt[L], 1)] = u0 + k * 256 + (int32_t)threadIdx.x;
  }
}
__global__ void __launch_bounds__(256) k_len_scatter(int32_t U, const int32_t *__restrict__ seed_read, const int32_t *__restrict__ len,
                                                     int32_t *__restrict__ cursor, int32_t lcap, int32_t *__restrict__ sorted_uniq)
{
  const int32_t stride = gridDim.x * blockDim.x;
  for (int32_t u0 = blockIdx.x * blockDim.x; u0 < U; u0 += stride) {
    const int32_t u = u0 + threadIdx.x;
    const bool ok = u < U;
    int L = ok ? len[seed_read[u]] : -1; if (L >= lcap) L = lcap - 1;
    unsigned long long todo = __ballot(ok);
    const unsigned long long below = (1ull << (threadIdx.x & 63)) - 1ull;
    while (todo) {
      const int leader = __ffsll((long long)todo) - 1;
      const int L0 = __shfl(L, leader, 64);
      const unsigned long long same = __ballot(ok && L == L0) & todo;
      int32_t base = 0;
      if ((int)(threadIdx.x & 63) == leader) base = atomicAdd(&cursor[L0], __popcll(same));
      base = __shfl(base, leader, 64);
      if (ok && L == L0 && (same >> (threadIdx.x & 63) & 1)) sorted_uniq[base + __popcll(same & below)] = u;
      todo &= ~same;
    }
  }
}

struct RegKey {
  const uint32_t *w; const uint32_t *exc; int nexc, nw_read, off, Ld, prof, L;
  int nwd, nex_in;
  __device__ __forceinline__ uint32_t word(int j) const
  {
    const int start = off + 16 * j;
    const int a = start >> 4, s = (start & 15) * 2;
    const uint32_t lo = w[a];
    const uint32_t up = (a + 1 < nw_read) ? w[a + 1] : 0u;
    uint32_t W = s ? ((lo >> s) | (up << (32 - s))) : lo;
    const int cnt = Ld - 16 * j;
    if (cnt < 16) W &= (1u << (2 * cnt)) - 1u;
    return W;
  }
  __device__ __forceinline__ uint32_t operator()(int j) const
  {
    if (j < nwd) return word(j);
    j -= nwd;
    if (j < nex_in) {
      int seen = 0;
      for (int e = 0; e < nexc; e++) {
        const int p = (int)(exc[e] >> 4);
        if (p >= off && p < off + Ld) { if (seen == j) return ((uint32_t)(p - off) << 4) | (exc[e] & 15u); seen++; }
      }
      return 0u;
    }
    j -= nex_in;
    return j == 0 ? (uint32_t)prof : j == 1 ? (uint32_t)L : (uint32_t)Ld;
  }
};
__device__ __forceinline__ RegKey make_regkey(const ReadsDev &rd, int read, int ienv, int jenv, int prof, int L)
{
  RegKey k;
  const int64_t wo = rd.woff[read], eo = rd.excoff[read];
  k.w = rd.words + wo; k.exc = rd.exc + eo; k.nexc = (int)(rd.excoff[read + 1] - eo); k.nw_read = (int)(rd.woff[read + 1] - wo);
  k.off = ienv - 1; k.Ld = jenv - ienv + 1; k.prof = prof; k.L = L;
  k.nwd = (k.Ld + 15) >> 4;
  int n = 0;
  for (int e = 0; e < k.nexc; e++) { const int p = (int)(k.exc[e] >> 4); n += (p >= k.off && p < k.off + k.Ld); }
  k.nex_in = n;
  return k;
}

__global__ void __launch_bounds__(256) k_region_keys(ReadsDev rd, const RegionRec *__restrict__ regions, int64_t nr, const PairRec *__restrict__ pairs,
                                                     const int32_t *__restrict__ sorted_uniq, const int32_t *__restrict__ seed_read,
                                                     unsigned long long *__restrict__ keys, int32_t *__restrict__ vals, uint64_t mask,
                                                     uint32_t *__restrict__ slot_of)
{
  for (int64_t g = (int64_t)blockIdx.x * blockDim.x + threadIdx.x; g < nr; g += (int64_t)gridDim.x * blockDim.x) {
    const RegionRec rg = regions[g];
    if (rg.pair < 0) { slot_of[g] = 0xFFFFFFFFu; continue; }
    const PairRec pr = pairs[rg.pair];
    const RegKey rk = make_regkey(rd, seed_read[sorted_uniq[pr.useq]], rg.ienv, rg.jenv, pr.prof, pr.L);
    uint64_t key = xxh64_words(rk, rk.nwd + rk.nex_in + 3, 0x9E3779B97F4A7C15ULL);
    if (key == 0) key = 1;
    uint64_t slot = (key * 0x9E3779B97F4A7C15ULL >> 20) & mask;
    for (;;) {
      const unsigned long long old = atomicCAS(&keys[slot], 0ull, (unsigned long long)key);
      if (old == 0ull || old == key) { atomicMin(&vals[slot], (int32_t)g); slot_of[g] = (uint32_t)slot; break; }
      slot = (slot + 1) & mask;
    }
  }
}
__global__ void __launch_bounds__(256) k_region_resolve(ReadsDev rd, const RegionRec *__restrict__ regions, int64_t nr, const PairRec *__restrict__ pairs,
                                                        const int32_t *__restrict__ sorted_uniq, const int32_t *__restrict__ seed_read,
                                                        const int32_t *__restrict__ vals, const uint32_t *__restrict__ slot_of,
                                                        int32_t *__restrict__ rep_region, int32_t *__restrict__ is_uniq)
{
  for (int64_t g = (int64_t)blockIdx.x * blockDim.x + threadIdx.x; g < nr; g += (int64_t)gridDim.x * blockDim.x) {
    const uint32_t slot = slot_of[g];
    if (slot == 0xFFFFFFFFu) { rep_region[g] = -1; is_uniq[g] = 0; continue; }
    int32_t s = vals[slot];
    if (s != (int32_t)g) {
      const RegionRec a = regions[g], b = regions[s];
      const PairRec pa = pairs[a.pair], pb = pairs[b.pair];
      bool same = pa.prof == pb.prof && pa.L == pb.L && (a.jenv - a.ienv) == (b.jenv - b.ienv);
      if (same) {
        const RegKey ka = make_regkey(rd, seed_read[sorted_uniq[pa.useq]], a.ienv, a.jenv, pa.prof, pa.L);
        const RegKey kb = make_regkey(rd, seed_read[sorted_uniq[pb.useq]], b.ienv, b.jenv, pb.prof, pb.L);
        same = ka.nex_in == kb.nex_in;
        for (int j = 0; same && j < ka.nwd + ka.nex_in; j++) same = ka(j) == kb(j);
      }
      if (!same) s = (int32_t)g;
    }
    rep_region[g] = s; is_uniq[g] = (s == (int32_t)g);
  }
}
__global__ void __launch_bounds__(256) k_region_upos(int64_t nr, const RegionRec *__restrict__ regions, const PairRec *__restrict__ pairs,
                                                     const int32_t *__restrict__ is_uniq, const int32_t *__restrict__ urank,
                                                     const int64_t *__restrict__ rseg, const int64_t *__restrict__ useg,
                                                     int32_t *__restrict__ upos, RegionRec *__restrict__ ulist)
{
  for (int64_t g = (int64_t)blockIdx.x * blockDim.x + threadIdx.x; g < nr; g += (int64_t)gridDim.x * blockDim.x) {
    if (!is_uniq[g]) continue;
    const RegionRec rg = regions[g];
    const int p = pairs[rg.pair].prof;
    const int64_t pos = useg[p] + (int64_t)(urank[g] - urank[rseg[p]]);
    upos[g] = (int32_t)pos;
    ulist[pos] = rg;
  }
}
__global__ void __launch_bounds__(256) k_region_upos_follow(int64_t nr, const int32_t *__restrict__ rep_region, const int32_t *__restrict__ is_uniq,
                                                            int32_t *__restrict__ upos)
{
  for (int64_t g = (int64_t)blockIdx.x * blockDim.x + threadIdx.x; g < nr; g += (int64_t)gridDim.x * blockDim.x) {
    const int32_t s = rep_region[g];
    if (s >= 0 && !is_uniq[g]) upos[g] = upos[s];
  }
}

static inline int grid_for(int64_t n, int block = 256, int cap = 8192)
{
  int64_t g = (n + block - 1) / block;
  if (g < 1) g = 1;
  if (g > cap) g = cap;
  return (int)g;
}

void launch_hash_reads(const ReadsDev &rd, uint64_t seed, int strand_both, uint64_t *hf, uint64_t *hr, hipStream_t st, const int32_t *sample)
{
  hipLaunchKernelGGL(k_hash_reads, dim3(grid_for(rd.n)), dim3(256), 0, st, rd, seed, strand_both, hf, hr, sample);
}
void launch_table_insert(int64_t n, const int32_t *len, int minlen, const uint64_t *hf, const uint64_t *hr,
                         unsigned long long *keys, int32_t *vals, uint64_t mask, uint32_t *slot_of, hipStream_t st)
{
  hipLaunchKernelGGL(k_table_insert, dim3(grid_for(n)), dim3(256), 0, st, n, len, minlen, hf, hr, keys, vals, mask, slot_of);
}
void launch_table_resolve(const ReadsDev &rd, const uint64_t *hf, const int32_t *vals, const uint32_t *slot_of,
                          int32_t *rep_of, int8_t *strand, int32_t *is_seed, unsigned int *n_collisions, hipStream_t st,
                          const int32_t *sample)
{
  hipLaunchKernelGGL(k_table_resolve, dim3(grid_for(rd.n)), dim3(256), 0, st, rd, hf, vals, slot_of, rep_of, strand, is_seed, n_collisions, sample);
}
void launch_uniques(int64_t n, const int32_t *rep_of, const int32_t *seed_rank, int32_t *uniq_of, int32_t *seed_read,
                    int32_t *abundance, hipStream_t st)
{
  hipLaunchKernelGGL(k_uniques, dim3(grid_for(n)), dim3(256), 0, st, n, rep_of, seed_rank, uniq_of, seed_read, abundance);
}
constexpr int LEN_LDS_BINS = 8192;
void launch_len_hist(int32_t U, const int32_t *seed_read, const int32_t *len, int32_t *hist, int32_t lcap, hipStream_t st, int32_t nb)
{
  if (nb > 0 && nb <= LEN_LDS_BINS && nb <= lcap)
    hipLaunchKernelGGL(k_len_bins<false>, dim3((unsigned)((U + LEN_TILE - 1) / LEN_TILE)), dim3(256), (size_t)nb * 4, st, U, seed_read, len, hist, nb, nullptr);
  else
    hipLaunchKernelGGL(k_len_hist, dim3(grid_for(U)), dim3(256), 0, st, U, seed_read, len, hist, lcap);
}
void launch_region_keys(const ReadsDev &rd, const RegionRec *regions, int64_t nr, const PairRec *pairs, const int32_t *sorted_uniq,
                        const int32_t *seed_read, unsigned long long *keys, int32_t *vals, uint64_t mask, uint32_t *slot_of, hipStream_t st)
{
  hipLaunchKernelGGL(k_region_keys, dim3(grid_for(nr)), dim3(256), 0, st, rd, regions, nr, pairs, sorted_uniq, seed_read, keys, vals, mask, slot_of);
}
void launch_region_resolve(const ReadsDev &rd, const RegionRec *regions, int64_t nr, const PairRec *pairs, const int32_t *sorted_uniq,
                           const int32_t *seed_read, const int32_t *vals, const uint32_t *slot_of, int32_t *rep_region, int32_t *is_uniq, hipStream_t st)
{
  hipLaunchKernelGGL(k_region_resolve, dim3(grid_for(nr)), dim3(256), 0, st, rd, regions, nr, pairs, sorted_uniq, seed_read, vals, slot_of, rep_region, is_uniq);
}
void launch_region_upos(int64_t nr, const RegionRec *regions, const PairRec *pairs, const int32_t *is_uniq, const int32_t *urank,
                        const int64_t *rseg, const int64_t *useg, int32_t *upos, RegionRec *ulist, hipStream_t st)
{
  hipLaunchKernelGGL(k_region_upos, dim3(grid_for(nr)), dim3(256), 0, st, nr, regions, pairs, is_uniq, urank, rseg, useg, upos, ulist);
}
void launch_region_upos_follow(int64_t nr, const int32_t *rep_region, const int32_t *is_uniq, int32_t *upos, hipStream_t st)
{
  hipLaunchKernelGGL(k_region_upos_follow, dim3(grid_for(nr)), dim3(256), 0, st, nr, rep_region, is_uniq, upos);
}
void launch_len_scatter(int32_t U, const int32_t *seed_read, const int32_t *len, int32_t *cursor, int32_t lcap,
                        int32_t *sorted_uniq, hipStream_t st, int32_t nb)
{
  if (nb > 0 && nb <= LEN_LDS_BINS && nb <= lcap)
    hipLaunchKernelGGL(k_len_bins<true>, dim3((unsigned)((U + LEN_TILE - 1) / LEN_TILE)), dim3(256), (size_t)nb * 8, st, U, seed_read, len, cursor, nb, sorted_uniq);
  else
    hipLaunchKernelGGL(k_len_scatter, dim3(grid_for(U)), dim3(256), 0, st, U, seed_read, len, cursor, lcap, sorted_uniq);
}

}
```

itsxpress_amd/csrc/k_ensemble.hip:

```cpp
#include "engine.h"
#include "k_api.h"
#include "detmath.h"
#include "k_vec.h"
#include <type_traits>

namespace itsx {

enum { tBM = 0, tMM, tIM, tDM, tMD, tMI, tII, tDD };
enum { ST_M = 1, ST_D, ST_I, ST_S, ST_N, ST_B, ST_E, ST_C, ST_T, ST_J };

DEV f4 *mrslab(const MrArgs &a, int64_t r0, int row, int v, int lane) { (void)lane; return (f4 *)a.slab + ((r0 + row) * MRV + v); }
constexpr int MR_SP = QMAX * 4 + 1, MR_CJ = QMAX * 4 + 2;
static_assert(MR_CJ < MRV, "matrix row too short");
DEV float comp4(const f4 &t, int r) { return r == 0 ? t.x : r == 1 ? t.y : r == 2 ? t.z : t.w; }
DEV f4 tof4(const V4 &v) { return (f4){v.a.x, v.a.y, v.b.x, v.b.y}; }

struct MrLane {
  bool active; int64_t mi, slot; MrRec m; int L, Lr, off, Q; const DevProfile *pp; Seq sq; float pmove, ploop; int64_t r0;
};
DEV MrLane mr_lane(const MrArgs &a, const WaveDesc &wd, int lane)
{
  MrLane e;
  e.active = lane < wd.count;
  const int64_t slot = wd.first + (e.active ? lane : 0);
// ... 584 lines not shown
        for (int x = 0; x < nm; x++) {
          const int h = Sstack[x];
          const Tup th = unpack_tup(Skey[h]);
          const int v = f == 0 ? th.i : f == 1 ? th.k : f == 2 ? th.j : th.m;
          Sepc[v - lo[f]] += Stcount[h];
        }
        for (int z = 0; z < W; z++) {
          const int w = Sepc[z];
          if (w >= thr && (pick < 0 || !leftmost)) pick = lo[f] + z;
          if (w > amw) { amw = w; am = lo[f] + z; }
        }
      } else {
        for (int x = 0; x < nm; x++) {
          const Tup th = unpack_tup(Skey[Sstack[x]]);
          const int v = f == 0 ? th.i : f == 1 ? th.k : f == 2 ? th.j : th.m;
          int w = 0;
          for (int y = 0; y < nm; y++) {
            const Tup tu = unpack_tup(Skey[Sstack[y]]);
            const int vu = f == 0 ? tu.i : f == 1 ? tu.k : f == 2 ? tu.j : tu.m;
            if (vu == v) w += Stcount[Sstack[y]];
          }
          if (w >= thr && (pick < 0 || (leftmost ? v < pick : v > pick))) pick = v;
          if (w > amw || (w == amw && v < am)) { amw = w; am = v; }
        }
      }
      best[f] = pick >= 0 ? pick : am;
    }
    if (best[0] > best[2] || best[1] > best[3]) continue;
    if (nsig >= capSig) { status = 6; break; }
    Ssig_i[nsig] = best[0]; Ssig_j[nsig] = best[2]; Ssig_p[nsig] = (float)ninc / (float)200;
    nsig++;
  }
  if (status == 0) {
    for (int x = 1; x < nsig; x++) {
      const int ti = Ssig_i[x], tj = Ssig_j[x]; const float tp = Ssig_p[x];
      int y = x - 1;
      while (y >= 0 && Ssig_i[y] > ti) { Ssig_i[y + 1] = Ssig_i[y]; Ssig_j[y + 1] = Ssig_j[y]; Ssig_p[y + 1] = Ssig_p[y]; y--; }
      Ssig_i[y + 1] = ti; Ssig_j[y + 1] = tj; Ssig_p[y + 1] = tp;
    }
    for (int d = 0; d < nsig; d++) Sdominated[d] = 0;
    for (int d = 0; d < nsig; d++)
      for (int d2 = d + 1; d2 < nsig; d2++) {
        const int nov = min(Ssig_j[d], Ssig_j[d2]) - max(Ssig_i[d], Ssig_i[d2]) + 1;
        if (nov == 0) break;
        const int n = min(Ssig_j[d] - Ssig_i[d] + 1, Ssig_j[d2] - Ssig_i[d2] + 1);
        if ((float)nov / (float)n >= 0.8f) { if (Ssig_p[d] > Ssig_p[d2]) Sdominated[d2] = 1; else Sdominated[d] = 1; }
      }
    for (int d = 0; d < nsig; d++) {
      if (Sdominated[d]) continue;
      if (out.nenv >= capEnv) { status = 7; break; }
      if (out.nenv < MRENV) { out.ei[out.nenv] = Ssig_i[d]; out.ej[out.nenv] = Ssig_j[d]; }
      if constexpr (BIG) { Senv[2 * out.nenv] = Ssig_i[d]; Senv[2 * out.nenv + 1] = Ssig_j[d]; }
      out.nenv++;
    }
  }
  if (status != 0) {
    out.nenv = 0;
    for (int pos = 0; pos < Lr; pos++) n2[pos] = 0.0f;
  }
  out.status = status;
  a.out[e.mi] = out;
  if (a.dbg && lane == 0) { atomicAdd(&a.dbg[0], tk_walk); atomicAdd(&a.dbg[1], tk_close); atomicAdd(&a.dbg[2], wall_clock64() - tk2); atomicAdd(&a.dbg[3], 1ull); atomicAdd(&a.dbg[4], tk_dedupe); }
}
#undef DOM_IJ
#undef DOM_KM

__global__ void __launch_bounds__(256) k_mr_count(const PairOut *__restrict__ pout, const RegionRec *__restrict__ raw, RegionPoolView pv, int64_t npairs,
                                                  int32_t *__restrict__ cnt)
{
  const int64_t pi = (int64_t)blockIdx.x * blockDim.x + threadIdx.x;
  if (pi > npairs) return;
  int c = 0;
  if (pi < npairs && pout[pi].pass_fwd)
    for (int k = 0; k < pout[pi].ndom; k++) c += raw_region(raw, pv, pi, k).multi != 0;
  cnt[pi] = c;
}
__global__ void __launch_bounds__(256) k_mr_fill(const PairOut *__restrict__ pout, const RegionRec *__restrict__ raw, RegionPoolView pv, int64_t npairs,
                                                 const int32_t *__restrict__ off, MrRec *__restrict__ mr)
{
  const int64_t pi = (int64_t)blockIdx.x * blockDim.x + threadIdx.x;
  if (pi >= npairs || !pout[pi].pass_fwd) return;
  int o = off[pi];
  for (int k = 0; k < pout[pi].ndom; k++) {
    const RegionRec r = raw_region(raw, pv, pi, k);
    if (!r.multi) continue;
    MrRec m; m.pair = (int32_t)pi; m.slot = k; m.ireg = r.ienv; m.jreg = r.jenv;
    mr[o++] = m;
  }
}
__global__ void __launch_bounds__(256) k_mr_ulist(int64_t nmr, const MrRec *__restrict__ mr, const int32_t *__restrict__ rep, const int32_t *__restrict__ is_uniq,
                                                  const int32_t *__restrict__ urank, int32_t *__restrict__ ulist, int32_t *__restrict__ ulen,
                                                  int32_t *__restrict__ mr_u)
{
  const int64_t m = (int64_t)blockIdx.x * blockDim.x + threadIdx.x;
  if (m >= nmr) return;
  const int32_t r = rep[m] >= 0 ? rep[m] : (int32_t)m;
  mr_u[m] = urank[r];
  if (is_uniq[m]) { ulist[urank[m]] = (int32_t)m; ulen[urank[m]] = mr[m].jreg - mr[m].ireg + 1; }
}
__global__ void __launch_bounds__(256) k_mr_reorder(int64_t nu, int64_t nmr, const int32_t *__restrict__ newpos, const int32_t *__restrict__ ulist_in,
                                                    int32_t *__restrict__ ulist_out, int32_t *__restrict__ mr_u)
{
  const int64_t x = (int64_t)blockIdx.x * blockDim.x + threadIdx.x;
  if (x < nu) ulist_out[newpos[x]] = ulist_in[x];
  if (x < nmr) mr_u[x] = newpos[mr_u[x]];
}
template <class Emit>
DEV int walk_region_list(const RegionListArgs &a, int64_t pi, int nraw, unsigned long long *nfail, unsigned long long *nenv, unsigned long long *kind, Emit emit)
{
  int n = 0, mk = a.mr_off ? a.mr_off[pi] : 0;
  for (int k = 0; k < nraw; k++) {
    const RegionRec r = raw_region(a.raw, a.pv, pi, k);
    if (!r.multi || !a.mr_off) { emit(n++, r); continue; }
    const MrOut o = a.mrout[a.mr_u[mk]];
    if (o.status != 0) {
      if (nfail) { (*nfail)++; kind[o.status & 7]++; }
      RegionRec c = r; c.multi = -1;
      emit(n++, c);
    } else {
      if (nenv) *nenv += (unsigned long long)o.nenv;
      const int32_t *env = o.big >= 0 ? a.envpool + o.big : nullptr;
      for (int z = 0; z < o.nenv; z++) {
        RegionRec c; c.pair = (int32_t)pi; c.multi = mk + 1;
        c.ienv = (env ? env[2 * z] : o.ei[z]) + r.ienv - 1; c.jenv = (env ? env[2 * z + 1] : o.ej[z]) + r.ienv - 1;
        emit(n++, c);
      }
    }
    mk++;
  }
  return n;
}
__global__ void __launch_bounds__(256) k_region_list_count(RegionListArgs a, int32_t *__restrict__ cnt, unsigned long long *__restrict__ counters)
{
  const int64_t pi = (int64_t)blockIdx.x * blockDim.x + threadIdx.x;
  if (pi > a.npairs) return;
  int n = 0;
  if (pi < a.npairs && a.pout[pi].pass_fwd) {
    unsigned long long nfail = 0, nenv = 0, kind[8] = {0, 0, 0, 0, 0, 0, 0, 0};
    n = walk_region_list(a, pi, a.pout[pi].ndom, &nfail, &nenv, kind, [](int, const RegionRec &) {});
    a.pout[pi].nregions_raw = a.pout[pi].ndom;
    a.pout[pi].ndom = n;
    if (nfail) { atomicAdd(&counters[0], nfail); for (int z = 1; z < 8; z++) if (kind[z]) atomicAdd(&counters[2 + z], kind[z]); }
    if (nenv) atomicAdd(&counters[1], nenv);
  }
  cnt[pi] = n;
}
__global__ void __launch_bounds__(256) k_region_list_fill(RegionListArgs a, const int64_t *__restrict__ pair_region0, RegionRec *__restrict__ out)
{
  const int64_t pi = (int64_t)blockIdx.x * blockDim.x + threadIdx.x;
  if (pi >= a.npairs || !a.pout[pi].pass_fwd) return;
  const int64_t o = pair_region0[pi];
  walk_region_list(a, pi, a.pout[pi].nregions_raw, nullptr, nullptr, nullptr, [&](int n, const RegionRec &r) { out[o + n] = r; });
}
__global__ void __launch_bounds__(256) k_mr_overflowed(const MrOut *__restrict__ out, int64_t nu, int32_t *__restrict__ list, unsigned long long *__restrict__ n)
{
  const int64_t u = (int64_t)blockIdx.x * blockDim.x + threadIdx.x;
  if (u >= nu) return;
  const int st = out[u].status;
  if (st == 2 || st == 3 || st == 4 || st == 6 || st == 7) list[atomicAdd(n, 1ULL)] = (int32_t)u;
}

void launch_mr_count(const PairOut *pout, const RegionRec *raw, RegionPoolView pv, int64_t npairs, int32_t *cnt, hipStream_t st)
{
  hipLaunchKernelGGL(k_mr_count, dim3((unsigned)((npairs + 1 + 255) / 256)), dim3(256), 0, st, pout, raw, pv, npairs, cnt);
}
void launch_mr_fill(const PairOut *pout, const RegionRec *raw, RegionPoolView pv, int64_t npairs, const int32_t *off, MrRec *mr, hipStream_t st)
{
  if (npairs <= 0) return;
  hipLaunchKernelGGL(k_mr_fill, dim3((unsigned)((npairs + 255) / 256)), dim3(256), 0, st, pout, raw, pv, npairs, off, mr);
}
void launch_region_list_count(const RegionListArgs &a, int32_t *cnt, unsigned long long *counters, hipStream_t st)
{
  hipLaunchKernelGGL(k_region_list_count, dim3((unsigned)((a.npairs + 1 + 255) / 256)), dim3(256), 0, st, a, cnt, counters);
}
void launch_region_list_fill(const RegionListArgs &a, const int64_t *pair_region0, RegionRec *out, hipStream_t st)
{
  if (a.npairs <= 0) return;
  hipLaunchKernelGGL(k_region_list_fill, dim3((unsigned)((a.npairs + 255) / 256)), dim3(256), 0, st, a, pair_region0, out);
}
void launch_mr_overflowed(const MrOut *out, int64_t nu, int32_t *list, unsigned long long *n, hipStream_t st)
{
  if (nu > 0) hipLaunchKernelGGL(k_mr_overflowed, dim3((unsigned)((nu + 255) / 256)), dim3(256), 0, st, out, nu, list, n);
}

void launch_mr_ulist(int64_t nmr, const MrRec *mr, const int32_t *rep, const int32_t *is_uniq, const int32_t *urank, int32_t *ulist, int32_t *ulen,
                     int32_t *mr_u, hipStream_t st)
{
  if (nmr <= 0) return;
  hipLaunchKernelGGL(k_mr_ulist, dim3((unsigned)((nmr + 255) / 256)), dim3(256), 0, st, nmr, mr, rep, is_uniq, urank, ulist, ulen, mr_u);
}
void launch_mr_reorder(int64_t nu, int64_t nmr, const int32_t *newpos, const int32_t *ulist_in, int32_t *ulist_out, int32_t *mr_u, hipStream_t st)
{
  const int64_t n = nu > nmr ? nu : nmr;
  if (n <= 0) return;
  hipLaunchKernelGGL(k_mr_reorder, dim3((unsigned)((n + 255) / 256)), dim3(256), 0, st, nu, nmr, newpos, ulist_in, ulist_out, mr_u);
}
void launch_mr_ensemble(const MrArgs &a, int nwaves, int wave0, hipStream_t st, int64_t one_first, int64_t one_count)
{
  if (nwaves <= 0) return;
  hipLaunchKernelGGL(k_mr_fwd, dim3(nwaves), dim3(64), 0, st, a, wave0);
  if (one_count > 0) hipLaunchKernelGGL((k_mr_trace<false, true>), dim3((unsigned)one_count), dim3(64), (size_t)a.lds_bytes, st, a, (int)one_first);
  else hipLaunchKernelGGL(k_mr_trace<false>, dim3(nwaves), dim3(64), 0, st, a, wave0);
}
void launch_mr_ensemble_big(const MrArgs &a, int nwaves, hipStream_t st)
{
  if (nwaves <= 0) return;
  hipLaunchKernelGGL(k_mr_fwd, dim3(nwaves), dim3(64), 0, st, a, 0);
  hipLaunchKernelGGL(k_mr_trace<true>, dim3(nwaves), dim3(64), 0, st, a, 0);
}
}
```

itsxpress_amd/csrc/switches.cpp:

```cpp
#include "switches.h"
#include <cstdlib>
#include <cstring>

namespace itsx {

static const Switch g_sw[] = {
  {"ITSX_NO_ENSEMBLE", SW_HOOK, "multidomain regions keep their region as one envelope instead of hmmsearch's stochastic-traceback clustering (changes envelopes)"},
  {"ITSX_LAZY_ZUB_SCALE", SW_HOOK, "multiplies the lazy stage's upper bound on domZ: more undecided rows for the completion tests"},
  {"ITSX_LAZY_FORCE_PENDING", SW_HOOK, "treats rows as undecided so that the completion path runs"},
  {"ITSX_LAZY_NO_RERUN", SW_HOOK, "skips the full re-search safety net (leaves undecided rows undecided)"},
  {"ITSX_LAZY_NO_COMPLETE", SW_HOOK, "skips itsx_lazy_complete inside itsx_search_finalize (leaves undecided rows undecided)"},
  {"ITSX_COMPACT_ZMAX", SW_HOOK, "largest domZ the compact / lazy modes call a row 'certain' for (default 1e9); a value below the data's domZ can drop a winner"},
  {"ITSX_COMPACT_DOME_MIN", SW_HOOK, "smallest --domE the compact / lazy modes call a row 'certain' for (default 1e-2)"},
  {"ITSX_PASSA_DBG", SW_HOOK, "pass A diagnostic bits (no rows / no restore / no join): timings only, scores are garbage"},
  {"ITSX_ROWS", SW_MODE, "rows mode when the caller did not call itsx_set_rows_mode: full | compact | lazy (coordinates identical in all three)"},
  {"ITSX_COMPACT_ROWS", SW_MODE, "=1: rows mode compact (older spelling of ITSX_ROWS=compact)"},
  {"ITSX_QMASK", SW_MODE, "=none: vsearch's --qmask none for cluster_size / orient seeds (default dust, as vsearch)"},
  {"ITSX_KEEP_TRACE", SW_MODE, "keeps per-pair filter traces for itsx_get_pairtraces (forces the compact path of a lazy search)"},
  {"ITSX_GZIP_LEVEL", SW_MODE, "deflate level of the trimmed-FASTQ writers (default 6; output bytes differ, records do not)"},
  {"ITSX_TEST_HOOKS", SW_DIAG, "=1: honour the HOOK switches above"},
  {"ITSX_SHARE_CHECK", SW_DIAG, "runs the unshared kernels beside the shared ones and counts differences (itsx_stats.share_mismatch, join_maxdiff)"},
  {"ITSX_LAZY_CHECK_BOUND", SW_DIAG, "compares pass A's scores with HMMER's own Forward arithmetic (itsx_stats.lazy_bound_maxdiff)"},
  {"ITSX_LAZY_HIST", SW_DIAG, "prints the histogram of round-2 candidates per group"},
  {"ITSX_PASSA_DUMP", SW_DIAG, "prints every pass-A launch's waves and wave-rows (scripts/passa_launches.py)"},
  {"ITSX_TRACE_ALLOC", SW_DIAG, "prints every hipMalloc / free with its time"},
  {"ITSX_CL_DEBUG", SW_DIAG, "clustering: prints per-window counters"},
  {"ITSX_MR_DEBUG", SW_DIAG, "ensemble stage: prints per-batch counters"},
  {"ITSX_SHARE", SW_TUNING, "=0: no prefix sharing (round 4's schedule)"},
  {"ITSX_SHARE_TWO", SW_TUNING, "=0: one-sided (prefix-only) sharing for pass A"},
  {"ITSX_MSV_TWO", SW_TUNING, "=0: the MSV filter keeps the one-sided (prefix-only) schedule when pass A shares two-sidedly"},
  {"ITSX_SHARE_B", SW_TUNING, "rows per block of the prefix / suffix trees (default 32)"},
  {"ITSX_SHARE_GB", SW_TUNING, "budget of the saved row states, GB"},
  {"ITSX_SHARE_MIN", SW_TUNING, "smallest shared-row fraction for which the shared schedule is used (default 0.10)"},
  {"ITSX_SHARE_FWD_STREAMS", SW_TUNING, "1 | 2 streams for pass A's batches"},
  {"ITSX_SHARE_MSV_STREAMS", SW_TUNING, "1 | 2 streams for the MSV filter's batches"},
  {"ITSX_NO_CHAINREC", SW_TUNING, "pass A reads a chain's data through the round-5 arrays instead of its 64-byte record (A/B)"},
  {"ITSX_BOUND_FOLD", SW_TUNING, "=0: pass A's plain recurrences instead of the folded ones (also switches two-sided sharing off)"},
  {"ITSX_BOUND_RESCALE_EXP", SW_TUNING, "power of ten at which pass A rescales a row (default 20)"},
  {"ITSX_LAZY_TOPUP", SW_TUNING, "=0: undecided rows go straight to the full count of their profiles (no top-up round); =2: the round also looks for unreported pairs among a profile's weakest (rows settled from above)"},
  {"ITSX_LAZY_EXACT_BOUND", SW_TUNING, "pass A through the HMMER-order Forward kernel (A/B)"},
  {"ITSX_CHUNK_UNIQUES", SW_TUNING, "representatives per search chunk"},
  {"ITSX_MSV_OVERLAP", SW_TUNING, "=0: the next chunk's MSV filter does not run beside the domain stage"},
  {"ITSX_MSV_PAD", SW_TUNING, "dynamic LDS of the overlapped MSV launch (an occupancy cap)"},
  {"ITSX_MSV_WHOLE", SW_TUNING, "=0: MSV stages 16 words at a time even when the whole read fits LDS"},
  {"ITSX_BIAS_OVERLAP", SW_TUNING, "=0: the bias filter does not run on the second stream"},
  {"ITSX_ST2_PRIO", SW_TUNING, "priority of the second stream"},
  {"ITSX_LOAD_PRIORITY", SW_TUNING, "=0: loads do not use the high-priority stream"},
  {"ITSX_SLAB_GB", SW_TUNING, "DP slab budget, GB"},
  {"ITSX_SLAB_ADAPT", SW_TUNING, "=0: the slab budget does not adapt to the job"},
  {"ITSX_DEFER_FREE_GB", SW_TUNING, "device memory kept on the deferred-free list, GB"},
  {"ITSX_MR_LONG_FRAC", SW_TUNING, "ensemble stage: share of regions taken as 'long'"},
  {"ITSX_MR_LONG_LANES", SW_TUNING, "ensemble stage: lanes per long region"},
  {"ITSX_MSV_BWD_WHOLE", SW_TUNING, "=1: the MSV filter's Backward chains copy their whole read to LDS first (A/B arm: same cells)"},
  {"ITSX_LAZY_TOPUP_ALL", SW_TUNING, "=0: a profile whose undecided rows need most of its pairs is left to the full count (itsx_lazy_complete) instead of taking all its unevaluated pairs in the top-up round (same rows)"},
  {"ITSX_MR_WAVES", SW_TUNING, "ensemble stage: waves a batch is spread over (lanes per wave = regions / this, 2 .. 64); 0 = waves of 64 lanes"},
  {"ITSX_MR_ONE_MAX", SW_TUNING, "ensemble stage: a batch of at most this many regions (default 2048) is walked one region per wave with the matrix in LDS; 0 = never"},
  {"ITSX_CL_NOSCORE", SW_TUNING, "clustering: skips the score-only pre-pass (A/B arm; the walk then aligns every candidate: same outcomes)"},
  {"ITSX_CL_NOPRECHECK", SW_TUNING, "clustering: skips the certificate pre-check (A/B arm: same outcomes)"},
  {"ITSX_CL_CAPACITY", SW_TUNING, "clustering: candidate-list capacity"},
  {"ITSX_CL_CCAP", SW_TUNING, "clustering: centroid capacity step"},
  {"ITSX_CL_HEAVY", SW_TUNING, "clustering: heavy-word split on / off"},
  {"ITSX_CL_HEAVY_MIN", SW_TUNING, "clustering: centroids a word needs to count as conserved"},
  {"ITSX_CL_ROWS", SW_TUNING, "clustering: alignment rows per lane"},
  {"ITSX_CL_WINDOW", SW_TUNING, "clustering: queries per speculative window"},
  {"ITSX_PACK_CHUNK", SW_TUNING, "reads per packing launch"},
  {"ITSX_PACK_ECAP", SW_TUNING, "initial capacity of the exception list"},
  {"ITSX_HUGEPAGES", SW_TUNING, "=0: host buffers without MADV_HUGEPAGE"},
  {"ITSX_IO_LIBDEFLATE", SW_TUNING, "=0: zlib instead of libdeflate when both are present"},
  {"ITSX_IO_THREADS", SW_TUNING, "host threads of the FASTQ readers / writers"},
  {"ITSX_IO_BLOCK_KB", SW_TUNING, "deflate unit of the block-parallel writer"},
  {"ITSX_PARALLEL_INFLATE", SW_TUNING, "=0: single-stream inflate"},
  {"ITSX_PINFLATE_CHUNK_KB", SW_TUNING, "chunk of the block-parallel inflater"},
  {"ITSX_PARSE_MIN_MB", SW_TUNING, "smallest text parsed on several threads"},
  {"ITSX_TEXT_CACHE_GB", SW_TUNING, "inflated-text cache, GB"},
  {"ITSX_WRITE_MIN_MB", SW_TUNING, "smallest output written by several threads"},
  {"ITSX_WRITE_UNIT_KB", SW_TUNING, "unit of the streamed writer"},
  {"ITSX_STREAM_RESERVE_MB", SW_TUNING, "streamed loads: first reservation"},
  {"ITSX_STREAM_RESERVE_X", SW_TUNING, "streamed loads: growth factor"},
};
static const int g_nsw = (int)(sizeof(g_sw) / sizeof(g_sw[0]));

const Switch *sw_registry(int *n) { if (n) *n = g_nsw; return g_sw; }

static bool hooks_on() { const char *e = sw_get("ITSX_TEST_HOOKS"); return e && atoi(e) == 1; }

const char *sw_get(const char *name)
{
  const char *v = getenv(name);
  if (!v) return nullptr;
  for (int i = 0; i < g_nsw; i++)
    if (strcmp(g_sw[i].name, name) == 0) return (g_sw[i].kind == SW_HOOK && !hooks_on()) ? nullptr : v;
  return nullptr;
}

std::string sw_report()
{
  std::string out;
  const bool on = hooks_on();
  for (int i = 0; i < g_nsw; i++) {
    const char *v = getenv(g_sw[i].name);
    if (!v) continue;
    out += g_sw[i].name; out += "="; out += v;
    if (g_sw[i].kind == SW_HOOK && !on) out += " (ignored: ITSX_TEST_HOOKS is not 1)";
    out += "\n";
  }
  return out;
}

}
```

Measured before the change: 4.607 million.

## Overlap ensemble stage on side stream with envelopes of plain regions

New measurement: 4.644 million (median of 6 runs). No clear change (+0.8%).

```diff
diff --git a/itsxpress_amd/csrc/engine.hip b/itsxpress_amd/csrc/engine.hip
--- a/itsxpress_amd/csrc/engine.hip
+++ b/itsxpress_amd/csrc/engine.hip
@@ -366,6 +366,7 @@
   DBuf<int32_t> w_mrcnt, w_mroff, w_mrlen, w_mrloff, w_mrrows, w_mrulist, w_mrulist2, w_mru; DBuf<int64_t> w_mrrowoff; DBuf<MrRec> w_mr; DBuf<MrOut> w_mrout; DBuf<int64_t> w_n2off; DBuf<float> w_n2sc, w_mrslab;
   DBuf<uint8_t> w_mrscratch; DBuf<WaveDesc> w_mrwaves;
   DBuf<RegionRec> w_pool, w_pool_sorted; DBuf<int32_t> w_pool_k; DBuf<unsigned long long> w_pool_n, w_pool_key; int64_t pool_cap = 0;
+  DBuf<RegionRec> w_cat; DBuf<int32_t> w_pcnt, w_ppref, w_tcnt, w_tpref, w_cat_of, w_upos_cat; DBuf<int64_t> w_pseg, w_tseg, w_useg2;
   DBuf<int32_t> w_mrsel; DBuf<int64_t> w_mrselrow; DBuf<MrBig> w_mrbig; DBuf<uint8_t> w_mrarena; DBuf<int32_t> w_mrenv; DBuf<WaveDesc> w_mrbigwaves;
   DBuf<int32_t> w_cl, w_cr;
   DBuf<int8_t> w_side; DBuf<unsigned long long> w_bl, w_br; DBuf<int32_t> w_uind, w_us, w_ue, w_ut, w_rs, w_re, w_rt, w_ri, w_uflag;
@@ -2187,6 +2188,113 @@
   StageTimer tm_dom(st);
   int64_t NMR = 0;
   const bool ensemble = !(sw_get("ITSX_NO_ENSEMBLE") && atoi(sw_get("ITSX_NO_ENSEMBLE")) != 0);
+  const bool mr_overlap = !(sw_get("ITSX_MR_OVERLAP") && atoi(sw_get("ITSX_MR_OVERLAP")) == 0);
+  const int64_t erow_bytes = 104 * 64 * 4;
+  LazyTimers elazy(st);
+  auto env_batches = [&](std::vector<WaveDesc> &rw, const std::vector<char> &rgen, const std::vector<int32_t> &rrows, int wbeg, int NRW) -> int {
+    DBuf<WaveDesc> &d_rw = ctx->w_rw;
+    int64_t ebudget = (int64_t)(slab_gb * (1 << 30)) / erow_bytes;
+    DBuf<float> &d_eslab = ctx->w_eslab; int64_t ealloc = (int64_t)(d_eslab.cap / (104 * 64));
+    if (adapt && !sw_get("ITSX_SLAB_GB")) {
+      int64_t total_rows = 0;
+      for (int w = wbeg; w < NRW; w++) total_rows += rrows[(size_t)w];
+      ebudget = std::min(ebudget, std::max(std::max(total_rows / 4 + 1, ((int64_t)2 << 30) / erow_bytes), ealloc));
+    }
+    int w0 = wbeg;
+    while (w0 < NRW) {
+      int w1 = w0; int64_t r = 0;
+      while (w1 < NRW && rgen[w1] == rgen[w0] && (w1 == w0 || r + rrows[w1] <= ebudget)) { rw[w1].slab = r; rw[w1].rows = rrows[w1]; r += rrows[w1]; w1++; }
+      if (r > ealloc) {
+        if (d_eslab.alloc((size_t)r * 104 * 64) != hipSuccess) {
+          (void)hipGetLastError();
+          ealloc = 0;
+          if (w1 - w0 <= 1) SET_ERR(ctx, ITSX_E_NOMEM, "no device memory left for the envelope slab of a single wave");
+          ebudget = std::max<int64_t>(r / 2, rrows[(size_t)w0]);
+          S.n_slab_shrinks++;
+          continue;
+        }
+        ealloc = r;
+      }
+      HIPCHK(hipMemcpyAsync(d_rw.p + w0, rw.data() + w0, (size_t)(w1 - w0) * sizeof(WaveDesc), hipMemcpyHostToDevice, st));
+      EnvArgs a{};
+      a.rd = ctx->rd; a.sorted_uniq = d_sorted; a.seed_read = ctx->d_seed_read.p; a.prof = ctx->d_prof.p; a.lt = ctx->d_lt.p;
+      a.pairs = pl.pairs; a.regions = ctx->d_ulist.p; a.rout = ctx->d_rout.p; a.waves = d_rw.p; a.slab = d_eslab.p;
+      { const size_t t = elazy.begin(&S.ms_env_kernel); launch_envelopes(a, w1 - w0, w0, rgen[w0], st); elazy.end(t); }
+      for (int w = w0; w < w1; w++) S.env_rows += (int64_t)(rrows[w] - 1) * rw[w].count;
+      w0 = w1;
+    }
+    return ITSX_OK;
+  };
+  auto env_waves = [&](const std::vector<int32_t> &utotal, const std::vector<int64_t> &useg, std::vector<WaveDesc> &rw, std::vector<char> &rgen, std::vector<int32_t> &rrows) -> int {
+    const int wbeg = (int)rw.size();
+    for (int pass = 0; pass < 2; pass++)
+      for (int p = 0; p < P; p++) {
+        if ((int)ctx->generic_q[p] != pass) continue;
+        for (int64_t k = 0; k < utotal[p]; k += 64) {
+          WaveDesc w{}; w.prof = p; w.first = useg[p] + k; w.count = (int32_t)std::min<int64_t>(64, utotal[p] - k);
+          rw.push_back(w); rgen.push_back((char)pass);
+        }
+      }
+    const int NRW = (int)rw.size();
+    DBuf<WaveDesc> &d_rw = ctx->w_rw; DBuf<int32_t> &d_rrows = ctx->w_rrows;
+    HIPCHK(upload(d_rw, rw, st)); HIPCHK(d_rrows.alloc((size_t)NRW));
+    rrows.resize((size_t)NRW);
+    if (NRW > wbeg) {
+      hipLaunchKernelGGL(k_wave_rows_regions, dim3((NRW - wbeg + 255) / 256), dim3(256), 0, st, d_rw.p + wbeg, NRW - wbeg, ctx->d_ulist.p, d_rrows.p + wbeg);
+      HIPCHK(hipMemcpyAsync(rrows.data() + wbeg, d_rrows.p + wbeg, (size_t)(NRW - wbeg) * 4, hipMemcpyDeviceToHost, st));
+      HIPCHK(hipStreamSynchronize(st));
+    }
+    return ITSX_OK;
+  };
+  int64_t n_env_unique_plain = 0;
+  struct { bool done = false; int64_t NRp = 0, NTcap = 0, NUp = 0, NT = 0; uint64_t tsize = 0; std::vector<WaveDesc> rw; std::vector<char> rgen; std::vector<int32_t> rrows, tb; } ps;
+  auto plain_phase = [&]() -> int {
+    DBuf<int32_t> &pcnt = ctx->w_pcnt, &ppref = ctx->w_ppref, &stmp = ctx->w_scan2, &d_b = ctx->w_b;
+    HIPCHK(pcnt.alloc((size_t)NP + 1)); HIPCHK(ppref.alloc((size_t)NP + 1)); HIPCHK(stmp.alloc((size_t)scan_tmp_elems(NP + 2)));
+    launch_plain_count(pl.pout, d_raw.p, pv, NP, pcnt.p, st);
+    launch_exclusive_scan(pcnt.p, ppref.p, NP + 1, stmp.p, st);
+    std::vector<int32_t> pb((size_t)P + 1);
+    HIPCHK(upload(ctx->w_idx, pl.seg_start, st)); HIPCHK(d_b.alloc((size_t)P + 1));
+    hipLaunchKernelGGL(k_gather_i32, dim3((P + 1 + 255) / 256), dim3(256), 0, st, ppref.p, ctx->w_idx.p, P + 1, d_b.p);
+    HIPCHK(hipMemcpyAsync(pb.data(), d_b.p, ((size_t)P + 1) * 4, hipMemcpyDeviceToHost, st));
+    HIPCHK(hipStreamSynchronize(st));
+    const int64_t NRp = pb[(size_t)P], NTcap = (int64_t)MRENV * NMR, NC = NRp + NTcap;
+    if (NRp <= 0 || NC > ((int64_t)48 << 20)) return ITSX_OK;
+    HIPCHK(ctx->w_cat.alloc((size_t)NC + 1));
+    launch_plain_fill(pl.pout, d_raw.p, pv, NP, ppref.p, ctx->w_cat.p, st);
+    DBuf<unsigned long long> &rkeys = ctx->w_keys; DBuf<int32_t> &rvals = ctx->w_vals; DBuf<uint32_t> &rslot = ctx->w_slot_of;
+    DBuf<int32_t> &rrep = ctx->w_rrep, &ruq = ctx->w_ruq, &rurank = ctx->w_rurank, &rscan = ctx->w_scan_tmp;
+    uint64_t tsize = 1024; while (tsize < (uint64_t)NC * 2 + 16) tsize <<= 1;
+    HIPCHK(rkeys.alloc(tsize)); HIPCHK(rvals.alloc(tsize)); HIPCHK(rslot.alloc((size_t)NC + 1));
+    HIPCHK(rrep.alloc((size_t)NC + 1)); HIPCHK(ruq.alloc((size_t)NC + 1)); HIPCHK(rurank.alloc((size_t)NC + 1));
+    HIPCHK(rscan.alloc((size_t)scan_tmp_elems(NC + 1))); HIPCHK(ctx->w_upos_cat.alloc((size_t)NC + 1));
+    HIPCHK(hipMemsetAsync(rkeys.p, 0, tsize * sizeof(unsigned long long), st));
+    HIPCHK(hipMemsetAsync(rvals.p, 0x7f, tsize * sizeof(int32_t), st));
+    HIPCHK(hipMemsetAsync(ruq.p, 0, ((size_t)NC + 1) * sizeof(int32_t), st));
+    launch_region_keys(ctx->rd, ctx->w_cat.p, NRp, pl.pairs, d_sorted, ctx->d_seed_read.p, rkeys.p, rvals.p, tsize - 1, rslot.p, st);
+    launch_region_resolve(ctx->rd, ctx->w_cat.p, NRp, pl.pairs, d_sorted, ctx->d_seed_read.p, rvals.p, rslot.p, rrep.p, ruq.p, st);
+    launch_exclusive_scan(ruq.p, rurank.p, NRp + 1, rscan.p, st);
+    std::vector<int64_t> pseg(pb.begin(), pb.end());
+    std::vector<int32_t> ub((size_t)P + 1);
+    HIPCHK(upload(ctx->w_pseg, pseg, st));
+    hipLaunchKernelGGL(k_gather_i32, dim3((P + 1 + 255) / 256), dim3(256), 0, st, rurank.p, ctx->w_pseg.p, P + 1, d_b.p);
+    HIPCHK(hipMemcpyAsync(ub.data(), d_b.p, ((size_t)P + 1) * 4, hipMemcpyDeviceToHost, st));
+    HIPCHK(hipStreamSynchronize(st));
+    std::vector<int64_t> useg((size_t)P + 1, 0);
+    std::vector<int32_t> utotal((size_t)P);
+    for (int p = 0; p < P; p++) { utotal[p] = ub[p + 1] - ub[p]; useg[p + 1] = useg[p] + ((int64_t)utotal[p] + 63) / 64 * 64; S.n_env_unique += utotal[p]; n_env_unique_plain += utotal[p]; }
+    const int64_t NUp = useg[P], NUcap = NUp + NTcap + 64 * (int64_t)P + 64;
+    HIPCHK(upload(ctx->w_useg, useg, st));
+    HIPCHK(ctx->d_ulist.alloc((size_t)NUcap)); HIPCHK(ctx->d_rout.alloc((size_t)NUcap));
+    HIPCHK(hipMemsetAsync(ctx->d_rout.p, 0, (size_t)NUcap * sizeof(RegionOut), st));
+    launch_region_upos(NRp, ctx->w_cat.p, pl.pairs, ruq.p, rurank.p, ctx->w_pseg.p, ctx->w_useg.p, ctx->w_upos_cat.p, ctx->d_ulist.p, st);
+    launch_region_upos_follow(NRp, rrep.p, ruq.p, ctx->w_upos_cat.p, st);
+    { const int rc = env_waves(utotal, useg, ps.rw, ps.rgen, ps.rrows); if (rc != ITSX_OK) return rc; }
+    { const int rc = env_batches(ps.rw, ps.rgen, ps.rrows, 0, (int)ps.rw.size()); if (rc != ITSX_OK) return rc; }
+    ps.NRp = NRp; ps.NTcap = NTcap; ps.NUp = NUp; ps.tsize = tsize; ps.done = true;
+    return ITSX_OK;
+  };
+  hipStream_t const st_main = st;
   if (ensemble) {
     DBuf<int32_t> &mrcnt = ctx->w_mrcnt, &mroff = ctx->w_mroff, &stmp = ctx->w_scan2;
     HIPCHK(mrcnt.alloc((size_t)NP + 2)); HIPCHK(mroff.alloc((size_t)NP + 2)); HIPCHK(stmp.alloc((size_t)scan_tmp_elems(NP + 2)));
@@ -2197,6 +2305,13 @@
     HIPCHK(hipStreamSynchronize(st));
     NMR = tot;
     if (NMR > 0) {
+      bool split = mr_overlap && pv.n == 0 && sw_get("ITSX_MR_DEBUG") == nullptr;
+      if (split && !ctx->st3) {
+        if (hipStreamCreateWithFlags(&ctx->st3, hipStreamNonBlocking) != hipSuccess) { (void)hipGetLastError(); ctx->st3 = nullptr; split = false; }
+        else { (void)hipEventCreateWithFlags(&ctx->ev_s3a, hipEventDisableTiming); (void)hipEventCreateWithFlags(&ctx->ev_s3b, hipEventDisableTiming); }
+      }
+      if (split) { HIPCHK(hipEventRecord(ctx->ev_s3a, st_main)); HIPCHK(hipStreamWaitEvent(ctx->st3, ctx->ev_s3a, 0)); }
+      hipStream_t st = split ? ctx->st3 : st_main;
       StageTimer tm_e(st);
       static_assert(sizeof(MrRec) == sizeof(RegionRec), "MrRec is handed to the region memoisation kernels as a RegionRec");
       HIPCHK(ctx->w_mr.alloc((size_t)NMR));
@@ -2294,6 +2409,7 @@
         }
         w0 = w1;
       }
+      if (split) { const int rc = plain_phase(); if (rc != ITSX_OK) return rc; }
       {
         HIPCHK(ctx->w_mrsel.alloc((size_t)NU + 1)); HIPCHK(ctx->w_pool_n.alloc(2));
         HIPCHK(hipMemsetAsync(ctx->w_pool_n.p + 1, 0, sizeof(unsigned long long), st));
@@ -2365,20 +2481,30 @@
     HIPCHK(d_c.alloc(16));
     HIPCHK(hipMemsetAsync(d_c.p, 0, 16 * sizeof(int64_t), st));
     launch_region_list_count(rl, d_rcnt.p, (unsigned long long *)d_c.p, st);
+  }
+  launch_exclusive_scan(d_rcnt.p, d_rpref.p, NP + 1, d_scan_tmp.p, st);
+  std::vector<int32_t> bound((size_t)2 * P + 2);
+  {
+    DBuf<int64_t> &d_idx = ctx->w_idx; DBuf<int32_t> &d_b = ctx->w_b;
+    HIPCHK(upload(d_idx, pl.seg_start, st)); HIPCHK(d_b.alloc((size_t)2 * P + 2));
+    hipLaunchKernelGGL(k_gather_i32, dim3((P + 1 + 255) / 256), dim3(256), 0, st, d_rpref.p, d_idx.p, P + 1, d_b.p);
+    if (ps.done) {
+      HIPCHK(ctx->w_tcnt.alloc((size_t)NP + 1)); HIPCHK(ctx->w_tpref.alloc((size_t)NP + 1));
+      launch_tail_count(d_rcnt.p, ctx->w_pcnt.p, NP + 1, ctx->w_tcnt.p, st);
+      launch_exclusive_scan(ctx->w_tcnt.p, ctx->w_tpref.p, NP + 1, d_scan_tmp.p, st);
+      hipLaunchKernelGGL(k_gather_i32, dim3((P + 1 + 255) / 256), dim3(256), 0, st, ctx->w_tpref.p, d_idx.p, P + 1, d_b.p + P + 1);
+    }
     int64_t hc[10] = {0};
-    HIPCHK(hipMemcpyAsync(hc, d_c.p, sizeof(hc), hipMemcpyDeviceToHost, st));
+    HIPCHK(hipMemcpyAsync(hc, ctx->w_counters.p, sizeof(hc), hipMemcpyDeviceToHost, st));
+    HIPCHK(hipMemcpyAsync(bound.data(), d_b.p, ((size_t)(ps.done ? 2 : 1) * (P + 1)) * 4, hipMemcpyDeviceToHost, st));
     HIPCHK(hipStreamSynchronize(st));
     S.n_mr_failed += hc[0]; S.n_mr_envelopes += hc[1];
     for (int k = 0; k < 8; k++) S.n_mr_fail_kind[k] += hc[2 + k];
-  }
-  launch_exclusive_scan(d_rcnt.p, d_rpref.p, NP + 1, d_scan_tmp.p, st);
-  std::vector<int32_t> bound((size_t)P + 1);
-  {
-    DBuf<int64_t> &d_idx = ctx->w_idx; DBuf<int32_t> &d_b = ctx->w_b;
-    HIPCHK(upload(d_idx, pl.seg_start, st)); HIPCHK(d_b.alloc((size_t)P + 1));
-    hipLaunchKernelGGL(k_gather_i32, dim3((P + 1 + 255) / 256), dim3(256), 0, st, d_rpref.p, d_idx.p, P + 1, d_b.p);
-    HIPCHK(hipMemcpyAsync(bound.data(), d_b.p, ((size_t)P + 1) * 4, hipMemcpyDeviceToHost, st));
-    HIPCHK(hipStreamSynchronize(st));
+    if (ps.done) {
+      ps.tb.assign(bound.begin() + P + 1, bound.end());
+      ps.NT = ps.tb[(size_t)P];
+      if (ps.NT > ps.NTcap) { ps.done = false; S.n_env_unique -= n_env_unique_plain; }
+    }
   }
   std::vector<int64_t> rseg((size_t)P + 1, 0);
   std::vector<int32_t> rtotal((size_t)P);
@@ -2395,83 +2521,68 @@
     launch_region_offsets(NP, pl.pairs, d_rpref.p, pl.d_seg_start, d_rseg.p, ctx->d_pair_region0.p, st);
     HIPCHK(hipMemsetAsync(ctx->d_regions.p, 0xFF, (size_t)NR * sizeof(RegionRec), st));
     launch_region_list_fill(rl, ctx->d_pair_region0.p, ctx->d_regions.p, st);
-    DBuf<unsigned long long> &rkeys = ctx->w_keys; DBuf<int32_t> &rvals = ctx->w_vals; DBuf<uint32_t> &rslot = ctx->w_slot_of;
-    DBuf<int32_t> &rrep = ctx->w_rrep, &ruq = ctx->w_ruq, &rurank = ctx->w_rurank, &rscan = ctx->w_scan_tmp;
-    uint64_t tsize = 1024; while (tsize < (uint64_t)NR * 2 + 16) tsize <<= 1;
-    HIPCHK(rkeys.alloc(tsize)); HIPCHK(rvals.alloc(tsize)); HIPCHK(rslot.alloc((size_t)NR + 1));
-    HIPCHK(rrep.alloc((size_t)NR + 1)); HIPCHK(ruq.alloc((size_t)NR + 1)); HIPCHK(rurank.alloc((size_t)NR + 1));
-    HIPCHK(rscan.alloc((size_t)scan_tmp_elems(NR + 1))); HIPCHK(ctx->d_upos.alloc((size_t)NR + 1));
-    HIPCHK(hipMemsetAsync(rkeys.p, 0, tsize * sizeof(unsigned long long), st));
-    HIPCHK(hipMemsetAsync(rvals.p, 0x7f, tsize * sizeof(int32_t), st));
-    HIPCHK(hipMemsetAsync(ruq.p, 0, ((size_t)NR + 1) * sizeof(int32_t), st));
-    launch_region_keys(ctx->rd, ctx->d_regions.p, NR, pl.pairs, d_sorted, ctx->d_seed_read.p, rkeys.p, rvals.p, tsize - 1, rslot.p, st);
-    launch_region_resolve(ctx->rd, ctx->d_regions.p, NR, pl.pairs, d_sorted, ctx->d_seed_read.p, rvals.p, rslot.p, rrep.p, ruq.p, st);
-    launch_exclusive_scan(ruq.p, rurank.p, NR + 1, rscan.p, st);
-    std::vector<int32_t> ub((size_t)P + 1);
-    {
-      DBuf<int64_t> &d_idx = ctx->w_idx; DBuf<int32_t> &d_b = ctx->w_b;
-      HIPCHK(upload(d_idx, rseg, st)); HIPCHK(d_b.alloc((size_t)P + 1));
-      hipLaunchKernelGGL(k_gather_i32, dim3((P + 1 + 255) / 256), dim3(256), 0, st, rurank.p, d_idx.p, P + 1, d_b.p);
-      HIPCHK(hipMemcpyAsync(ub.data(), d_b.p, ((size_t)P + 1) * 4, hipMemcpyDeviceToHost, st));
-      HIPCHK(hipStreamSynchronize(st));
-    }
-    std::vector<int64_t> useg((size_t)P + 1, 0);
-    std::vector<int32_t> utotal((size_t)P);
-    for (int p = 0; p < P; p++) { utotal[p] = ub[p + 1] - ub[p]; useg[p + 1] = useg[p] + ((int64_t)utotal[p] + 63) / 64 * 64; S.n_env_unique += utotal[p]; }
-    const int64_t NU = useg[P];
-    DBuf<int64_t> &d_useg = ctx->w_useg;
-    HIPCHK(upload(d_useg, useg, st));
-    HIPCHK(ctx->d_ulist.alloc((size_t)std::max<int64_t>(NU, 1))); HIPCHK(ctx->d_rout.alloc((size_t)std::max<int64_t>(NU, 1)));
-    HIPCHK(hipMemsetAsync(ctx->d_rout.p, 0, (size_t)std::max<int64_t>(NU, 1) * sizeof(RegionOut), st));
-    launch_region_upos(NR, ctx->d_regions.p, pl.pairs, ruq.p, rurank.p, d_rseg.p, d_useg.p, ctx->d_upos.p, ctx->d_ulist.p, st);
-    launch_region_upos_follow(NR, rrep.p, ruq.p, ctx->d_upos.p, st);
-    std::vector<WaveDesc> rw; std::vector<char> rgen;
-    for (int pass = 0; pass < 2; pass++)
-      for (int p = 0; p < P; p++) {
-        if ((int)ctx->generic_q[p] != pass) continue;
-        for (int64_t k = 0; k < utotal[p]; k += 64) {
-          WaveDesc w{}; w.prof = p; w.first = useg[p] + k; w.count = (int32_t)std::min<int64_t>(64, utotal[p] - k);
-          rw.push_back(w); rgen.push_back((char)pass);
-        }
+    if (ps.done) {
+      const int64_t NRp = ps.NRp, NT = ps.NT;
+      DBuf<int32_t> &rrep = ctx->w_rrep, &ruq = ctx->w_ruq, &rurank = ctx->w_rurank, &rscan = ctx->w_scan_tmp;
+      HIPCHK(ctx->w_cat_of.alloc((size_t)NR)); HIPCHK(ctx->d_upos.alloc((size_t)NR + 1));
+      HIPCHK(hipMemsetAsync(ctx->w_cat_of.p, 0xFF, (size_t)NR * 4, st));
+      launch_region_list_split(rl, ctx->d_pair_region0.p, ctx->w_ppref.p, ctx->w_tpref.p, NRp, ctx->w_cat.p, ctx->w_cat_of.p, st);
+      if (NT > 0) {
+        launch_region_keys(ctx->rd, ctx->w_cat.p, NRp + NT, pl.pairs, d_sorted, ctx->d_seed_read.p, ctx->w_keys.p, ctx->w_vals.p, ps.tsize - 1, ctx->w_slot_of.p, st, NRp);
+        launch_region_resolve(ctx->rd, ctx->w_cat.p, NRp + NT, pl.pairs, d_sorted, ctx->d_seed_read.p, ctx->w_vals.p, ctx->w_slot_of.p, rrep.p, ruq.p, st, NRp);
+        launch_exclusive_scan(ruq.p + NRp, rurank.p + NRp, NT + 1, rscan.p, st);
+        std::vector<int64_t> tseg(ps.tb.begin(), ps.tb.end());
+        std::vector<int32_t> ub((size_t)P + 1);
+        DBuf<int32_t> &d_b = ctx->w_b;
+        HIPCHK(upload(ctx->w_tseg, tseg, st));
+        hipLaunchKernelGGL(k_gather_i32, dim3((P + 1 + 255) / 256), dim3(256), 0, st, rurank.p + NRp, ctx->w_tseg.p, P + 1, d_b.p);
+        HIPCHK(hipMemcpyAsync(ub.data(), d_b.p, ((size_t)P + 1) * 4, hipMemcpyDeviceToHost, st));
+        HIPCHK(hipStreamSynchronize(st));
+        std::vector<int64_t> useg((size_t)P + 1, ps.NUp);
+        std::vector<int32_t> utotal((size_t)P);
+        for (int p = 0; p < P; p++) { utotal[p] = ub[p + 1] - ub[p]; useg[p + 1] = useg[p] + ((int64_t)utotal[p] + 63) / 64 * 64; S.n_env_unique += utotal[p]; }
+        HIPCHK(upload(ctx->w_useg2, useg, st));
+        launch_region_upos(NT, ctx->w_cat.p + NRp, pl.pairs, ruq.p + NRp, rurank.p + NRp, ctx->w_tseg.p, ctx->w_useg2.p, ctx->w_upos_cat.p + NRp, ctx->d_ulist.p, st);
+        launch_region_upos_follow(NRp + NT, rrep.p, ruq.p, ctx->w_upos_cat.p, st, NRp);
+        const int wbeg = (int)ps.rw.size();
+        { const int rc = env_waves(utotal, useg, ps.rw, ps.rgen, ps.rrows); if (rc != ITSX_OK) return rc; }
+        { const int rc = env_batches(ps.rw, ps.rgen, ps.rrows, wbeg, (int)ps.rw.size()); if (rc != ITSX_OK) return rc; }
       }
-    const int NRW = (int)rw.size();
-    DBuf<WaveDesc> &d_rw = ctx->w_rw; DBuf<int32_t> &d_rrows = ctx->w_rrows;
-    HIPCHK(upload(d_rw, rw, st)); HIPCHK(d_rrows.alloc((size_t)NRW));
-    hipLaunchKernelGGL(k_wave_rows_regions, dim3((NRW + 255) / 256), dim3(256), 0, st, d_rw.p, NRW, ctx->d_ulist.p, d_rrows.p);
-    std::vector<int32_t> rrows((size_t)NRW);
-    HIPCHK(hipMemcpyAsync(rrows.data(), d_rrows.p, (size_t)NRW * 4, hipMemcpyDeviceToHost, st));
-    HIPCHK(hipStreamSynchronize(st));
-    const int64_t erow_bytes = 104 * 64 * 4;
-    int64_t ebudget = (int64_t)(slab_gb * (1 << 30)) / erow_bytes;
-    LazyTimers elazy(st);
-    DBuf<float> &d_eslab = ctx->w_eslab; int64_t ealloc = (int64_t)(d_eslab.cap / (104 * 64));
-    if (adapt && !sw_get("ITSX_SLAB_GB")) {
-      int64_t total_rows = 0;
-      for (int w = 0; w < NRW; w++) total_rows += rrows[(size_t)w];
-      ebudget = std::min(ebudget, std::max(std::max(total_rows / 4 + 1, ((int64_t)2 << 30) / erow_bytes), ealloc));
-    }
-    int w0 = 0;
-    while (w0 < NRW) {
-      int w1 = w0; int64_t r = 0;
-      while (w1 < NRW && rgen[w1] == rgen[w0] && (w1 == w0 || r + rrows[w1] <= ebudget)) { rw[w1].slab = r; rw[w1].rows = rrows[w1]; r += rrows[w1]; w1++; }
-      if (r > ealloc) {
-        if (d_eslab.alloc((size_t)r * 104 * 64) != hipSuccess) {
-          (void)hipGetLastError();
-          ealloc = 0;
-          if (w1 - w0 <= 1) SET_ERR(ctx, ITSX_E_NOMEM, "no device memory left for the envelope slab of a single wave");
-          ebudget = std::max<int64_t>(r / 2, rrows[(size_t)w0]);
-          S.n_slab_shrinks++;
-          continue;
-        }
-        ealloc = r;
+      launch_upos_final(NR, ctx->w_cat_of.p, ctx->w_upos_cat.p, ctx->d_upos.p, st);
+    } else {
+      DBuf<unsigned long long> &rkeys = ctx->w_keys; DBuf<int32_t> &rvals = ctx->w_vals; DBuf<uint32_t> &rslot = ctx->w_slot_of;
+      DBuf<int32_t> &rrep = ctx->w_rrep, &ruq = ctx->w_ruq, &rurank = ctx->w_rurank, &rscan = ctx->w_scan_tmp;
+      uint64_t tsize = 1024; while (tsize < (uint64_t)NR * 2 + 16) tsize <<= 1;
+      HIPCHK(rkeys.alloc(tsize)); HIPCHK(rvals.alloc(tsize)); HIPCHK(rslot.alloc((size_t)NR + 1));
+      HIPCHK(rrep.alloc((size_t)NR + 1)); HIPCHK(ruq.alloc((size_t)NR + 1)); HIPCHK(rurank.alloc((size_t)NR + 1));
+      HIPCHK(rscan.alloc((size_t)scan_tmp_elems(NR + 1))); HIPCHK(ctx->d_upos.alloc((size_t)NR + 1));
+      HIPCHK(hipMemsetAsync(rkeys.p, 0, tsize * sizeof(unsigned long long), st));
+      HIPCHK(hipMemsetAsync(rvals.p, 0x7f, tsize * sizeof(int32_t), st));
+      HIPCHK(hipMemsetAsync(ruq.p, 0, ((size_t)NR + 1) * sizeof(int32_t), st));
+      launch_region_keys(ctx->rd, ctx->d_regions.p, NR, pl.pairs, d_sorted, ctx->d_seed_read.p, rkeys.p, rvals.p, tsize - 1, rslot.p, st);
+      launch_region_resolve(ctx->rd, ctx->d_regions.p, NR, pl.pairs, d_sorted, ctx->d_seed_read.p, rvals.p, rslot.p, rrep.p, ruq.p, st);
+      launch_exclusive_scan(ruq.p, rurank.p, NR + 1, rscan.p, st);
+      std::vector<int32_t> ub((size_t)P + 1);
+      {
+        DBuf<int64_t> &d_idx = ctx->w_idx; DBuf<int32_t> &d_b = ctx->w_b;
+        HIPCHK(upload(d_idx, rseg, st)); HIPCHK(d_b.alloc((size_t)P + 1));
+        hipLaunchKernelGGL(k_gather_i32, dim3((P + 1 + 255) / 256), dim3(256), 0, st, rurank.p, d_idx.p, P + 1, d_b.p);
+        HIPCHK(hipMemcpyAsync(ub.data(), d_b.p, ((size_t)P + 1) * 4, hipMemcpyDeviceToHost, st));
+        HIPCHK(hipStreamSynchronize(st));
       }
-      HIPCHK(hipMemcpyAsync(d_rw.p + w0, rw.data() + w0, (size_t)(w1 - w0) * sizeof(WaveDesc), hipMemcpyHostToDevice, st));
-      EnvArgs a{};
-      a.rd = ctx->rd; a.sorted_uniq = d_sorted; a.seed_read = ctx->d_seed_read.p; a.prof = ctx->d_prof.p; a.lt = ctx->d_lt.p;
-      a.pairs = pl.pairs; a.regions = ctx->d_ulist.p; a.rout = ctx->d_rout.p; a.waves = d_rw.p; a.slab = d_eslab.p;
-      { const size_t t = elazy.begin(&S.ms_env_kernel); launch_envelopes(a, w1 - w0, w0, rgen[w0], st); elazy.end(t); }
-      for (int w = w0; w < w1; w++) S.env_rows += (int64_t)(rrows[w] - 1) * rw[w].count;
-      w0 = w1;
+      std::vector<int64_t> useg((size_t)P + 1, 0);
+      std::vector<int32_t> utotal((size_t)P);
+      for (int p = 0; p < P; p++) { utotal[p] = ub[p + 1] - ub[p]; useg[p + 1] = useg[p] + ((int64_t)utotal[p] + 63) / 64 * 64; S.n_env_unique += utotal[p]; }
+      const int64_t NU = useg[P];
+      DBuf<int64_t> &d_useg = ctx->w_useg;
+      HIPCHK(upload(d_useg, useg, st));
+      HIPCHK(ctx->d_ulist.alloc((size_t)std::max<int64_t>(NU, 1))); HIPCHK(ctx->d_rout.alloc((size_t)std::max<int64_t>(NU, 1)));
+      HIPCHK(hipMemsetAsync(ctx->d_rout.p, 0, (size_t)std::max<int64_t>(NU, 1) * sizeof(RegionOut), st));
+      launch_region_upos(NR, ctx->d_regions.p, pl.pairs, ruq.p, rurank.p, d_rseg.p, d_useg.p, ctx->d_upos.p, ctx->d_ulist.p, st);
+      launch_region_upos_follow(NR, rrep.p, ruq.p, ctx->d_upos.p, st);
+      std::vector<WaveDesc> rw; std::vector<char> rgen; std::vector<int32_t> rrows;
+      { const int rc = env_waves(utotal, useg, rw, rgen, rrows); if (rc != ITSX_OK) return rc; }
+      { const int rc = env_batches(rw, rgen, rrows, 0, (int)rw.size()); if (rc != ITSX_OK) return rc; }
     }
     ScoreArgs sa{};
     sa.rd = ctx->rd; sa.sorted_uniq = d_sorted; sa.seed_read = ctx->d_seed_read.p; sa.prof = ctx->d_prof.p; sa.lt = ctx->d_lt.p;
@@ -2480,6 +2591,7 @@
     if (NMR > 0) { sa.mr = ctx->w_mr.p; sa.mr_u = ctx->w_mru.p; sa.mrout = ctx->w_mrout.p; sa.n2off = ctx->w_n2off.p; sa.n2sc = ctx->w_n2sc.p; sa.mr_off = ctx->w_mroff.p; }
     sa.domz = ctx->d_domz32.p; sa.usample = ctx->dev_usample(); sa.P = ctx->P;
     launch_score(sa, st);
+    elazy.collect();
     if (ctx->compact_rows) {
       launch_compact_best(d_dom.p, NR, ctx->w_cls.p, ctx->compact_ncls, ctx->compact_lnp, ctx->w_bestc.p, st);
       HIPCHK(ctx->w_keep.alloc((size_t)NR + 1)); HIPCHK(ctx->w_keeppos.alloc((size_t)NR + 1)); HIPCHK(ctx->w_keeptmp.alloc((size_t)scan_tmp_elems(NR + 1)));
diff --git a/itsxpress_amd/csrc/k_api.h b/itsxpress_amd/csrc/k_api.h
--- a/itsxpress_amd/csrc/k_api.h
+++ b/itsxpress_amd/csrc/k_api.h
@@ -26,12 +26,12 @@
                         int32_t *sorted_uniq, hipStream_t st, int32_t nb = 0);
 
 void launch_region_keys(const ReadsDev &rd, const RegionRec *regions, int64_t nr, const PairRec *pairs, const int32_t *sorted_uniq,
-                        const int32_t *seed_read, unsigned long long *keys, int32_t *vals, uint64_t mask, uint32_t *slot_of, hipStream_t st);
+                        const int32_t *seed_read, unsigned long long *keys, int32_t *vals, uint64_t mask, uint32_t *slot_of, hipStream_t st, int64_t g0 = 0);
 void launch_region_resolve(const ReadsDev &rd, const RegionRec *regions, int64_t nr, const PairRec *pairs, const int32_t *sorted_uniq,
-                           const int32_t *seed_read, const int32_t *vals, const uint32_t *slot_of, int32_t *rep_region, int32_t *is_uniq, hipStream_t st);
+                           const int32_t *seed_read, const int32_t *vals, const uint32_t *slot_of, int32_t *rep_region, int32_t *is_uniq, hipStream_t st, int64_t g0 = 0);
 void launch_region_upos(int64_t nr, const RegionRec *regions, const PairRec *pairs, const int32_t *is_uniq, const int32_t *urank,
                         const int64_t *rseg, const int64_t *useg, int32_t *upos, RegionRec *ulist, hipStream_t st);
-void launch_region_upos_follow(int64_t nr, const int32_t *rep_region, const int32_t *is_uniq, int32_t *upos, hipStream_t st);
+void launch_region_upos_follow(int64_t nr, const int32_t *rep_region, const int32_t *is_uniq, int32_t *upos, hipStream_t st, int64_t g0 = 0);
 
 struct ClusterArgs {
   ReadsDev rd;
@@ -384,6 +384,12 @@
 };
 void launch_region_list_count(const RegionListArgs &a, int32_t *cnt, unsigned long long *counters, hipStream_t st);
 void launch_region_list_fill(const RegionListArgs &a, const int64_t *pair_region0, RegionRec *out, hipStream_t st);
+void launch_plain_count(const PairOut *pout, const RegionRec *raw, RegionPoolView pv, int64_t npairs, int32_t *cnt, hipStream_t st);
+void launch_plain_fill(const PairOut *pout, const RegionRec *raw, RegionPoolView pv, int64_t npairs, const int32_t *off, RegionRec *out, hipStream_t st);
+void launch_tail_count(const int32_t *cnt_final, const int32_t *cnt_plain, int64_t n, int32_t *cnt_tail, hipStream_t st);
+void launch_region_list_split(const RegionListArgs &a, const int64_t *pair_region0, const int32_t *plain_off, const int32_t *tail_off, int64_t nplain,
+                              RegionRec *cat, int32_t *cat_of, hipStream_t st);
+void launch_upos_final(int64_t nr, const int32_t *cat_of, const int32_t *upos_cat, int32_t *upos, hipStream_t st);
 
 struct ScoreArgs {
   ReadsDev rd;
diff --git a/itsxpress_amd/csrc/k_derep.hip b/itsxpress_amd/csrc/k_derep.hip
--- a/itsxpress_amd/csrc/k_derep.hip
+++ b/itsxpress_amd/csrc/k_derep.hip
@@ -317,9 +317,9 @@
 __global__ void __launch_bounds__(256) k_region_keys(ReadsDev rd, const RegionRec *__restrict__ regions, int64_t nr, const PairRec *__restrict__ pairs,
                                                      const int32_t *__restrict__ sorted_uniq, const int32_t *__restrict__ seed_read,
                                                      unsigned long long *__restrict__ keys, int32_t *__restrict__ vals, uint64_t mask,
-                                                     uint32_t *__restrict__ slot_of)
-{
-  for (int64_t g = (int64_t)blockIdx.x * blockDim.x + threadIdx.x; g < nr; g += (int64_t)gridDim.x * blockDim.x) {
+                                                     uint32_t *__restrict__ slot_of, int64_t g0)
+{
+  for (int64_t g = g0 + (int64_t)blockIdx.x * blockDim.x + threadIdx.x; g < nr; g += (int64_t)gridDim.x * blockDim.x) {
     const RegionRec rg = regions[g];
     if (rg.pair < 0) { slot_of[g] = 0xFFFFFFFFu; continue; }
     const PairRec pr = pairs[rg.pair];
@@ -337,9 +337,9 @@
 __global__ void __launch_bounds__(256) k_region_resolve(ReadsDev rd, const RegionRec *__restrict__ regions, int64_t nr, const PairRec *__restrict__ pairs,
                                                         const int32_t *__restrict__ sorted_uniq, const int32_t *__restrict__ seed_read,
                                                         const int32_t *__restrict__ vals, const uint32_t *__restrict__ slot_of,
-                                                        int32_t *__restrict__ rep_region, int32_t *__restrict__ is_uniq)
-{
-  for (int64_t g = (int64_t)blockIdx.x * blockDim.x + threadIdx.x; g < nr; g += (int64_t)gridDim.x * blockDim.x) {
+                                                        int32_t *__restrict__ rep_region, int32_t *__restrict__ is_uniq, int64_t g0)
+{
+  for (int64_t g = g0 + (int64_t)blockIdx.x * blockDim.x + threadIdx.x; g < nr; g += (int64_t)gridDim.x * blockDim.x) {
     const uint32_t slot = slot_of[g];
     if (slot == 0xFFFFFFFFu) { rep_region[g] = -1; is_uniq[g] = 0; continue; }
     int32_t s = vals[slot];
@@ -373,9 +373,9 @@
   }
 }
 __global__ void __launch_bounds__(256) k_region_upos_follow(int64_t nr, const int32_t *__restrict__ rep_region, const int32_t *__restrict__ is_uniq,
-                                                            int32_t *__restrict__ upos)
-{
-  for (int64_t g = (int64_t)blockIdx.x * blockDim.x + threadIdx.x; g < nr; g += (int64_t)gridDim.x * blockDim.x) {
+                                                            int32_t *__restrict__ upos, int64_t g0)
+{
+  for (int64_t g = g0 + (int64_t)blockIdx.x * blockDim.x + threadIdx.x; g < nr; g += (int64_t)gridDim.x * blockDim.x) {
     const int32_t s = rep_region[g];
     if (s >= 0 && !is_uniq[g]) upos[g] = upos[s];
   }
@@ -418,23 +418,23 @@
     hipLaunchKernelGGL(k_len_hist, dim3(grid_for(U)), dim3(256), 0, st, U, seed_read, len, hist, lcap);
 }
 void launch_region_keys(const ReadsDev &rd, const RegionRec *regions, int64_t nr, const PairRec *pairs, const int32_t *sorted_uniq,
-                        const int32_t *seed_read, unsigned long long *keys, int32_t *vals, uint64_t mask, uint32_t *slot_of, hipStream_t st)
-{
-  hipLaunchKernelGGL(k_region_keys, dim3(grid_for(nr)), dim3(256), 0, st, rd, regions, nr, pairs, sorted_uniq, seed_read, keys, vals, mask, slot_of);
+                        const int32_t *seed_read, unsigned long long *keys, int32_t *vals, uint64_t mask, uint32_t *slot_of, hipStream_t st, int64_t g0)
+{
+  hipLaunchKernelGGL(k_region_keys, dim3(grid_for(nr - g0)), dim3(256), 0, st, rd, regions, nr, pairs, sorted_uniq, seed_read, keys, vals, mask, slot_of, g0);
 }
 void launch_region_resolve(const ReadsDev &rd, const RegionRec *regions, int64_t nr, const PairRec *pairs, const int32_t *sorted_uniq,
-                           const int32_t *seed_read, const int32_t *vals, const uint32_t *slot_of, int32_t *rep_region, int32_t *is_uniq, hipStream_t st)
-{
-  hipLaunchKernelGGL(k_region_resolve, dim3(grid_for(nr)), dim3(256), 0, st, rd, regions, nr, pairs, sorted_uniq, seed_read, vals, slot_of, rep_region, is_uniq);
+                           const int32_t *seed_read, const int32_t *vals, const uint32_t *slot_of, int32_t *rep_region, int32_t *is_uniq, hipStream_t st, int64_t g0)
+{
+  hipLaunchKernelGGL(k_region_resolve, dim3(grid_for(nr - g0)), dim3(256), 0, st, rd, regions, nr, pairs, sorted_uniq, seed_read, vals, slot_of, rep_region, is_uniq, g0);
 }
 void launch_region_upos(int64_t nr, const RegionRec *regions, const PairRec *pairs, const int32_t *is_uniq, const int32_t *urank,
                         const int64_t *rseg, const int64_t *useg, int32_t *upos, RegionRec *ulist, hipStream_t st)
 {
   hipLaunchKernelGGL(k_region_upos, dim3(grid_for(nr)), dim3(256), 0, st, nr, regions, pairs, is_uniq, urank, rseg, useg, upos, ulist);
 }
-void launch_region_upos_follow(int64_t nr, const int32_t *rep_region, const int32_t *is_uniq, int32_t *upos, hipStream_t st)
-{
-  hipLaunchKernelGGL(k_region_upos_follow, dim3(grid_for(nr)), dim3(256), 0, st, nr, rep_region, is_uniq, upos);
+void launch_region_upos_follow(int64_t nr, const int32_t *rep_region, const int32_t *is_uniq, int32_t *upos, hipStream_t st, int64_t g0)
+{
+  hipLaunchKernelGGL(k_region_upos_follow, dim3(grid_for(nr - g0)), dim3(256), 0, st, nr, rep_region, is_uniq, upos, g0);
 }
 void launch_len_scatter(int32_t U, const int32_t *seed_read, const int32_t *len, int32_t *cursor, int32_t lcap,
                         int32_t *sorted_uniq, hipStream_t st, int32_t nb)
diff --git a/itsxpress_amd/csrc/k_ensemble.hip b/itsxpress_amd/csrc/k_ensemble.hip
--- a/itsxpress_amd/csrc/k_ensemble.hip
+++ b/itsxpress_amd/csrc/k_ensemble.hip
@@ -760,6 +760,51 @@
   const int64_t o = pair_region0[pi];
   walk_region_list(a, pi, a.pout[pi].nregions_raw, nullptr, nullptr, nullptr, [&](int n, const RegionRec &r) { out[o + n] = r; });
 }
+__global__ void __launch_bounds__(256) k_plain_count(const PairOut *__restrict__ pout, const RegionRec *__restrict__ raw, RegionPoolView pv, int64_t npairs,
+                                                     int32_t *__restrict__ cnt)
+{
+  const int64_t pi = (int64_t)blockIdx.x * blockDim.x + threadIdx.x;
+  if (pi > npairs) return;
+  int c = 0;
+  if (pi < npairs && pout[pi].pass_fwd)
+    for (int k = 0; k < pout[pi].ndom; k++) c += raw_region(raw, pv, pi, k).multi == 0;
+  cnt[pi] = c;
+}
+__global__ void __launch_bounds__(256) k_plain_fill(const PairOut *__restrict__ pout, const RegionRec *__restrict__ raw, RegionPoolView pv, int64_t npairs,
+                                                    const int32_t *__restrict__ off, RegionRec *__restrict__ out)
+{
+  const int64_t pi = (int64_t)blockIdx.x * blockDim.x + threadIdx.x;
+  if (pi >= npairs || !pout[pi].pass_fwd) return;
+  int64_t o = off[pi];
+  for (int k = 0; k < pout[pi].ndom; k++) {
+    const RegionRec r = raw_region(raw, pv, pi, k);
+    if (!r.multi) out[o++] = r;
+  }
+}
+__global__ void __launch_bounds__(256) k_tail_count(const int32_t *__restrict__ cnt_final, const int32_t *__restrict__ cnt_plain, int64_t n, int32_t *__restrict__ cnt_tail)
+{
+  const int64_t i = (int64_t)blockIdx.x * blockDim.x + threadIdx.x;
+  if (i < n) cnt_tail[i] = cnt_final[i] - cnt_plain[i];
+}
+__global__ void __launch_bounds__(256) k_region_list_split(RegionListArgs a, const int64_t *__restrict__ pair_region0, const int32_t *__restrict__ plain_off,
+                                                           const int32_t *__restrict__ tail_off, int64_t nplain, RegionRec *__restrict__ cat, int32_t *__restrict__ cat_of)
+{
+  const int64_t pi = (int64_t)blockIdx.x * blockDim.x + threadIdx.x;
+  if (pi >= a.npairs || !a.pout[pi].pass_fwd) return;
+  const int64_t o = pair_region0[pi];
+  int64_t np = plain_off[pi], nt = nplain + tail_off[pi];
+  walk_region_list(a, pi, a.pout[pi].nregions_raw, nullptr, nullptr, nullptr, [&](int n, const RegionRec &r) {
+    if (r.multi == 0) cat_of[o + n] = (int32_t)np++;
+    else { cat[nt] = r; cat_of[o + n] = (int32_t)nt++; }
+  });
+}
+__global__ void __launch_bounds__(256) k_upos_final(int64_t nr, const int32_t *__restrict__ cat_of, const int32_t *__restrict__ upos_cat, int32_t *__restrict__ upos)
+{
+  const int64_t g = (int64_t)blockIdx.x * blockDim.x + threadIdx.x;
+  if (g >= nr) return;
+  const int32_t c = cat_of[g];
+  if (c >= 0) upos[g] = upos_cat[c];
+}
 __global__ void __launch_bounds__(256) k_mr_overflowed(const MrOut *__restrict__ out, int64_t nu, int32_t *__restrict__ list, unsigned long long *__restrict__ n)
 {
   const int64_t u = (int64_t)blockIdx.x * blockDim.x + threadIdx.x;
@@ -786,6 +831,29 @@
   if (a.npairs <= 0) return;
   hipLaunchKernelGGL(k_region_list_fill, dim3((unsigned)((a.npairs + 255) / 256)), dim3(256), 0, st, a, pair_region0, out);
 }
+void launch_plain_count(const PairOut *pout, const RegionRec *raw, RegionPoolView pv, int64_t npairs, int32_t *cnt, hipStream_t st)
+{
+  hipLaunchKernelGGL(k_plain_count, dim3((unsigned)((npairs + 1 + 255) / 256)), dim3(256), 0, st, pout, raw, pv, npairs, cnt);
+}
+void launch_plain_fill(const PairOut *pout, const RegionRec *raw, RegionPoolView pv, int64_t npairs, const int32_t *off, RegionRec *out, hipStream_t st)
+{
+  if (npairs <= 0) return;
+  hipLaunchKernelGGL(k_plain_fill, dim3((unsigned)((npairs + 255) / 256)), dim3(256), 0, st, pout, raw, pv, npairs, off, out);
+}
+void launch_tail_count(const int32_t *cnt_final, const int32_t *cnt_plain, int64_t n, int32_t *cnt_tail, hipStream_t st)
+{
+  if (n > 0) hipLaunchKernelGGL(k_tail_count, dim3((unsigned)((n + 255) / 256)), dim3(256), 0, st, cnt_final, cnt_plain, n, cnt_tail);
+}
+void launch_region_list_split(const RegionListArgs &a, const int64_t *pair_region0, const int32_t *plain_off, const int32_t *tail_off, int64_t nplain,
+                              RegionRec *cat, int32_t *cat_of, hipStream_t st)
+{
+  if (a.npairs <= 0) return;
+  hipLaunchKernelGGL(k_region_list_split, dim3((unsigned)((a.npairs + 255) / 256)), dim3(256), 0, st, a, pair_region0, plain_off, tail_off, nplain, cat, cat_of);
+}
+void launch_upos_final(int64_t nr, const int32_t *cat_of, const int32_t *upos_cat, int32_t *upos, hipStream_t st)
+{
+  if (nr > 0) hipLaunchKernelGGL(k_upos_final, dim3((unsigned)((nr + 255) / 256)), dim3(256), 0, st, nr, cat_of, upos_cat, upos);
+}
 void launch_mr_overflowed(const MrOut *out, int64_t nu, int32_t *list, unsigned long long *n, hipStream_t st)
 {
   if (nu > 0) hipLaunchKernelGGL(k_mr_overflowed, dim3((unsigned)((nu + 255) / 256)), dim3(256), 0, st, out, nu, list, n);
diff --git a/itsxpress_amd/csrc/switches.cpp b/itsxpress_amd/csrc/switches.cpp
--- a/itsxpress_amd/csrc/switches.cpp
+++ b/itsxpress_amd/csrc/switches.cpp
@@ -54,6 +54,7 @@
   {"ITSX_MSV_BWD_WHOLE", SW_TUNING, "=1: the MSV filter's Backward chains copy their whole read to LDS first (A/B arm: same cells)"},
   {"ITSX_LAZY_TOPUP_ALL", SW_TUNING, "=0: a profile whose undecided rows need most of its pairs is left to the full count (itsx_lazy_complete) instead of taking all its unevaluated pairs in the top-up round (same rows)"},
   {"ITSX_MR_WAVES", SW_TUNING, "ensemble stage: waves a batch is spread over (lanes per wave = regions / this, 2 .. 64); 0 = waves of 64 lanes"},
+  {"ITSX_MR_OVERLAP", SW_TUNING, "=0: the ensemble stage does not run on a side stream beside the envelopes of the regions that are not multidomain (the serial order: same rows)"},
   {"ITSX_MR_ONE_MAX", SW_TUNING, "ensemble stage: a batch of at most this many regions (default 2048) is walked one region per wave with the matrix in LDS; 0 = never"},
   {"ITSX_CL_NOSCORE", SW_TUNING, "clustering: skips the score-only pre-pass (A/B arm; the walk then aligns every candidate: same outcomes)"},
   {"ITSX_CL_NOPRECHECK", SW_TUNING, "clustering: skips the certificate pre-check (A/B arm: same outcomes)"},
```
